# eridgd/WCT-TF

Hardware: AMD Instinct MI355X
Metric: stylized frames/sec @512x512, 5-level relu5->1 pipeline, alpha=0.8 (higher is better)
Workload: dtype f16

## Files before the change

include/wct_hip.h:

```cpp
#ifndef WCT_HIP_H
#define WCT_HIP_H

#include <stddef.h>
#include <stdint.h>

#ifdef __cplusplus
extern "C" {
#endif

typedef struct wct_ctx wct_ctx;

enum wct_status { WCT_STATUS_OK = 0, WCT_STATUS_HIP = -1, WCT_STATUS_ARG = -2,
                  WCT_STATUS_STATE = -3, WCT_STATUS_NOMEM = -4,
                  WCT_STATUS_NOCONV = -5 };

enum wct_mode { WCT_NP = 0, WCT_TF = 1 };

enum wct_flags {
  WCT_FLAG_ADAIN = 1,
  WCT_FLAG_MODE_NP = 2,
  WCT_FLAG_SWAP5 = 4,
  WCT_FLAG_STYLE_SHARED = 8,
  WCT_FLAG_IMAGES_F32 = 16,
  WCT_FLAG_CONTENT_COLORS = 32,
  WCT_FLAG_GUIDED = 64
};

int  wct_create(int device, wct_ctx** out);
void wct_destroy(wct_ctx* ctx);
const char* wct_last_error(void);
int  wct_sync(wct_ctx* ctx);
int  wct_device_count(int* n);
int  wct_get_stream(wct_ctx* ctx, void** stream_out);

int wct_set_encoder(wct_ctx* ctx, const float* pre_w, const float* pre_b,
                    const float* const* w, const float* const* b, int n_layers);
int wct_set_decoder(wct_ctx* ctx, int level, const float* const* w, const float* const* b,
                    int n_layers);

int wct_transform(wct_ctx* ctx, const float* content, int Nc, const float* style, int Ns,
                  int C, float alpha, int mode, float eps, float* out,
                  int* sweeps_out );
int wct_adain(wct_ctx* ctx, const float* content, int Nc, const float* style, int Ns,
              int C, float alpha, float epsilon, float* out);
int wct_transform_mix(wct_ctx* ctx, const float* content, int Nc, const float* const* styles, const int* Ns, int K,
                      const float* weights, int C, float alpha, int mode, float eps, float* out, int* sweeps_out);
int wct_adain_mix(wct_ctx* ctx, const float* content, int Nc, const float* const* styles, const int* Ns, int K,
                  const float* weights, int C, float alpha, float epsilon, float* out);
int wct_transform_masked(wct_ctx* ctx, const float* content, int Nc, const uint8_t* labels, const float* const* styles,
                         const int* Ns, int K, int C, float alpha, int mode, float eps, float* out, int* sweeps_out);
int wct_adain_masked(wct_ctx* ctx, const float* content, int Nc, const uint8_t* labels, const float* const* styles,
                     const int* Ns, int K, int C, float alpha, float epsilon, float* out);
int wct_mask_compact(wct_ctx* ctx, const uint8_t* mask, int Hm, int Wm, int h, int w, int stride, int K, int* perm_out,
                     int* seg_off_out);
int wct_mask_compact_batch(wct_ctx* ctx, const uint8_t* masks, int B, int Hm, int Wm, int h, int w, int stride, int K,
                           int* perm_out, int* seg_off_out);
int wct_style_swap(wct_ctx* ctx, const float* content, int hc, int wc, const float* style, int hs, int ws,
                   int C, float alpha, int patch_size, int stride, float eps, float* out);
int wct_set_style_swap(wct_ctx* ctx, float ss_alpha, int patch_size, int stride);
int wct_eigh(wct_ctx* ctx, const float* A, int C, int nmat, float* evals, float* evecs,
             int* sweeps_out );
int wct_conv3x3(wct_ctx* ctx, const float* x, int H, int W, int Cin, const float* w_hwio,
                const float* bias, int Cout, int relu, int upsample, float* y);
int wct_conv3x3_f16(wct_ctx* ctx, const float* x, int B, int H, int W, int Cin, const float* w_hwio,
                    const float* bias, int Cout, int relu, int upsample, int pool, int algo, float* y);
int wct_maxpool(wct_ctx* ctx, const float* x, int H, int W, int C, float* y);
int wct_encode(wct_ctx* ctx, const float* img01, int H, int W, int level, float* feat);
int wct_decode(wct_ctx* ctx, const float* feat, int h, int w, int level, float* img);
int wct_coral_stats(wct_ctx* ctx, const uint8_t* img, int H, int W, double sums[9]);
int wct_coral_apply(wct_ctx* ctx, const uint8_t* src, int H, int W, const double M[9],
                    const double src_mean[3], const double src_std[3],
                    const double tgt_mean[3], const double tgt_std[3],
                    uint8_t* out_u8, double* out_f64);
int wct_content_colors(wct_ctx* ctx, const uint8_t* stylized, int Ho, int Wo, const uint8_t* content, int Hc, int Wc,
                       uint8_t* out);
int wct_content_colors_batch_dev(wct_ctx* ctx, const uint8_t* stylized_dev, int Ho, int Wo, const uint8_t* content_dev, int Hc,
                                 int Wc, int B, uint8_t* out_dev);
int wct_guided_filter(wct_ctx* ctx, const uint8_t* stylized, int Ho, int Wo, const uint8_t* content, int Hc, int Wc, int radius,
                      int eps_q, uint8_t* out);
int wct_guided_filter_batch_dev(wct_ctx* ctx, const uint8_t* stylized_dev, int Ho, int Wo, const uint8_t* content_dev, int Hc, int Wc,
                                int B, int radius, int eps_q, uint8_t* out_dev);
int wct_set_guided(wct_ctx* ctx, int radius, int eps_q);
int wct_resize(wct_ctx* ctx, const uint8_t* img, int H, int W, int h, int w, uint8_t* out);
int wct_resize_batch_dev(wct_ctx* ctx, const uint8_t* in_dev, int H, int W, int B, int h, int w, uint8_t* out_dev);

int wct_output_size(int Hc, int Wc, const int* levels, int n_levels, int* Ho, int* Wo);
int wct_stylize(wct_ctx* ctx, const uint8_t* content, int Hc, int Wc,
                const uint8_t* style, int Hs, int Ws,
                const int* levels, int n_levels, float alpha, unsigned flags,
                uint8_t* out);
int wct_stylize_mix(wct_ctx* ctx, const uint8_t* content, int Hc, int Wc, const uint8_t* const* styles, const int* Hs,
                    const int* Ws, int K, const float* weights, const int* levels, int n_levels, float alpha, unsigned flags,
                    uint8_t* out);
int wct_stylize_masked(wct_ctx* ctx, const uint8_t* content, int Hc, int Wc, const uint8_t* mask, const uint8_t* const* styles,
                       const int* Hs, const int* Ws, int K, const int* levels, int n_levels, float alpha, unsigned flags,
                       uint8_t* out);
int wct_stylize_batch_dev(wct_ctx* ctx, const uint8_t* content_dev, int Hc, int Wc,
                          const uint8_t* style_dev, int Hs, int Ws, int B,
                          const int* levels, int n_levels, float alpha, unsigned flags,
                          uint8_t* out_dev);

typedef struct wct_style wct_style;
int  wct_style_prepare(wct_ctx* ctx, const uint8_t* style, int Hs, int Ws, const int* levels, int n_levels, unsigned flags,
                       wct_style** out);
void wct_style_free(wct_ctx* ctx, wct_style* style);
int  wct_stylize_prepared(wct_ctx* ctx, const uint8_t* content, int Hc, int Wc, const wct_style* style, const int* levels,
                          int n_levels, float alpha, unsigned flags, uint8_t* out);
int  wct_stylize_prepared_batch_dev(wct_ctx* ctx, const uint8_t* content_dev, int Hc, int Wc, int B, const wct_style* style,
                                    const int* levels, int n_levels, float alpha, unsigned flags, uint8_t* out_dev);
int  wct_stylize_prepared_mix(wct_ctx* ctx, const uint8_t* content, int Hc, int Wc, const wct_style* const* styles, int K,
                              const float* weights, const int* levels, int n_levels, float alpha, unsigned flags,
                              uint8_t* out);
int  wct_stylize_prepared_masked(wct_ctx* ctx, const uint8_t* content, int Hc, int Wc, const uint8_t* mask,
                                 const wct_style* const* styles, int K, const int* levels, int n_levels, float alpha,
                                 unsigned flags, uint8_t* out);
int  wct_stylize_prepared_masked_batch_dev(wct_ctx* ctx, const uint8_t* content_dev, int Hc, int Wc, int B,
                                           const uint8_t* masks_host, const wct_style* const* styles, int K, const int* levels,
                                           int n_levels, float alpha, unsigned flags, uint8_t* out_dev);

typedef struct wct_warm wct_warm;
int  wct_warm_create(wct_ctx* ctx, const int* levels, int n_levels, wct_warm** out);
void wct_warm_free(wct_ctx* ctx, wct_warm* warm);
int  wct_warm_reset(wct_ctx* ctx, wct_warm* warm);
int  wct_warm_basis(wct_ctx* ctx, const wct_warm* warm, int level, int* valid, float* V_host );
int  wct_stylize_prepared_warm(wct_ctx* ctx, const uint8_t* content, int Hc, int Wc, const wct_style* style, const int* levels,
                               int n_levels, float alpha, unsigned flags, wct_warm* warm, uint8_t* out);
int  wct_stylize_prepared_batch_dev_warm(wct_ctx* ctx, const uint8_t* content_dev, int Hc, int Wc, int B, const wct_style* style,
                                         const int* levels, int n_levels, float alpha, unsigned flags, wct_warm* warm,
                                         uint8_t* out_dev);
int  wct_transform_warm(wct_ctx* ctx, const float* content, int Nc, const float* style, int Ns, int C, float alpha,
                        unsigned flags, wct_warm* warm, int level, float* out, int* sweeps_out);

int  wct_transform_strength(wct_ctx* ctx, const float* content, int Nc, int h, int w, const uint8_t* smap, int Hm, int Wm,
                            int stride, const float* style, int Ns, int C, float alpha, int mode, float eps, float* out,
                            int* sweeps_out );
int  wct_adain_strength(wct_ctx* ctx, const float* content, int Nc, int h, int w, const uint8_t* smap, int Hm, int Wm, int stride,
                        const float* style, int Ns, int C, float alpha, float epsilon, float* out);
int  wct_stylize_prepared_strength(wct_ctx* ctx, const uint8_t* content, int Hc, int Wc, const uint8_t* smap, const wct_style* style,
                                   const int* levels, int n_levels, float alpha, unsigned flags, uint8_t* out);
int  wct_stylize_prepared_strength_batch_dev(wct_ctx* ctx, const uint8_t* content_dev, int Hc, int Wc, int B,
                                             const uint8_t* smaps_dev , const wct_style* style, const int* levels,
                                             int n_levels, float alpha, unsigned flags, uint8_t* out_dev);
int  wct_stylize_prepared_strength_batch_dev_warm(wct_ctx* ctx, const uint8_t* content_dev, int Hc, int Wc, int B,
                                                  const uint8_t* smaps_dev, const wct_style* style, const int* levels, int n_levels,
                                                  float alpha, unsigned flags, wct_warm* warm, uint8_t* out_dev);

int wct_texture_noise_batch_dev(wct_ctx* ctx, int H, int W, int B, unsigned seed, unsigned first_sample, int smooth,
                                uint8_t* out_dev);
int wct_texture_noise(wct_ctx* ctx, int H, int W, unsigned seed, unsigned sample, int smooth, uint8_t* out_host);
int wct_texture_size(int H, int W, const int* levels, int n_levels, int passes, int* Ho, int* Wo);
int wct_texture_prepared_batch_dev(wct_ctx* ctx, int H, int W, int B, unsigned seed, unsigned first_sample, int smooth,
                                   const wct_style* style, const int* levels, int n_levels, int passes, float alpha,
                                   unsigned flags, uint8_t* out_dev);
int wct_texture_prepared(wct_ctx* ctx, int H, int W, unsigned seed, unsigned sample, int smooth,
                         const wct_style* style, const int* levels, int n_levels, int passes, float alpha,
                         unsigned flags, uint8_t* out_host);

int wct_band_rows(int Hc, int Wc, const int* levels, int n_levels, int* band_rows);
int wct_band_plan(int H, int W, int level, int band_rows, int max_bands, int* n_bands, int* rows );
int wct_encode_banded(wct_ctx* ctx, const float* img01, int H, int W, int level, int band_rows, float* feat);
int wct_decode_banded(wct_ctx* ctx, const float* feat, int h, int w, int level, int band_rows, float* img);
int wct_transform_chunked(wct_ctx* ctx, const float* content, int Nc, const float* style, int Ns, int C, float alpha, int mode,
                          float eps, int chunk_rows, float* out, int* sweeps_out);
int wct_stylize_prepared_banded_dev(wct_ctx* ctx, const uint8_t* content_dev, int Hc, int Wc, const wct_style* style,
                                    const int* levels, int n_levels, float alpha, unsigned flags, int band_rows, int stat_rows,
                                    uint8_t* out_dev);
int wct_stylize_prepared_banded(wct_ctx* ctx, const uint8_t* content, int Hc, int Wc, const wct_style* style, const int* levels,
                                int n_levels, float alpha, unsigned flags, int band_rows, int stat_rows, uint8_t* out);

int wct_wrap_halo(int level, int* enc, int* dec_before, int* dec_after);
int wct_wrap_check(int H, int W, const int* levels, int n_levels);
int wct_wrap_pad_batch_dev(wct_ctx* ctx, const float* in_dev, int B, int H, int W, int C, int top, int bottom, int left, int right,
                           float* out_dev);
int wct_wrap_pad(wct_ctx* ctx, const float* x, int H, int W, int C, int top, int bottom, int left, int right, float* y);
int wct_encode_wrap(wct_ctx* ctx, const float* img01, int H, int W, int level, float* feat);
int wct_decode_wrap(wct_ctx* ctx, const float* feat, int h, int w, int level, float* img);
int wct_stylize_prepared_wrap_batch_dev(wct_ctx* ctx, const uint8_t* content_dev, int Hc, int Wc, int B, const wct_style* style,
                                        const int* levels, int n_levels, float alpha, unsigned flags, uint8_t* out_dev);
int wct_stylize_prepared_wrap(wct_ctx* ctx, const uint8_t* content, int Hc, int Wc, const wct_style* style, const int* levels,
                              int n_levels, float alpha, unsigned flags, uint8_t* out);
int wct_texture_prepared_wrap_batch_dev(wct_ctx* ctx, int H, int W, int B, unsigned seed, unsigned first_sample, int smooth,
                                        const wct_style* style, const int* levels, int n_levels, int passes, float alpha,
                                        unsigned flags, uint8_t* out_dev);
int wct_texture_prepared_wrap(wct_ctx* ctx, int H, int W, unsigned seed, unsigned sample, int smooth,
                              const wct_style* style, const int* levels, int n_levels, int passes, float alpha,
                              unsigned flags, uint8_t* out_host);

int wct_train_step(wct_ctx* ctx, int level, const float* images, int B, int H, int W,
                   float feature_weight, float pixel_weight, float tv_weight,
                   float lr, float beta1, float beta2, float eps, int step, float* losses_out);
int wct_get_decoder_layer(wct_ctx* ctx, int level, int layer, float* w_hwio, float* bias,
                          float* grad_w, float* grad_b);

int wct_train_grad_buffer(wct_ctx* ctx, int level, float** grad_dev, size_t* count);
int wct_train_apply(wct_ctx* ctx, int level, float lr, float beta1, float beta2, float eps, int step);

int wct_dev_alloc(wct_ctx* ctx, size_t bytes, void** out);
int wct_dev_free(wct_ctx* ctx, void* p);
int wct_h2d(wct_ctx* ctx, void* dst_dev, const void* src_host, size_t bytes);
int wct_d2h(wct_ctx* ctx, void* dst_host, const void* src_dev, size_t bytes);

#define WCT_PROF_CLASSES 11
int wct_prof_enable(wct_ctx* ctx, int on);
int wct_prof_reset(wct_ctx* ctx);
int wct_prof_read(wct_ctx* ctx, double ms[WCT_PROF_CLASSES], long long launches[WCT_PROF_CLASSES],
                  double flops[WCT_PROF_CLASSES], double bytes[WCT_PROF_CLASSES]);
int wct_eig_stats(wct_ctx* ctx, long long out[18]);

#ifdef __cplusplus
}
#endif
#endif
```

wct_tf_amd/_lib.py:

```python
import ctypes as C
import os

import numpy as np

_HERE = os.path.dirname(os.path.abspath(__file__))
LIB_PATH = os.path.join(_HERE, 'libwct_hip.so')

_P = C.c_void_p
_F = C.POINTER(C.c_float)
_I = C.POINTER(C.c_int)
_U8 = C.POINTER(C.c_uint8)
_D = C.POINTER(C.c_double)
_PP = C.POINTER(C.c_void_p)
SIGNATURES = [
    ('wct_create', C.c_int, [C.c_int, _PP]),
    ('wct_destroy', None, [_P]),
    ('wct_last_error', C.c_char_p, []),
    ('wct_sync', C.c_int, [_P]),
    ('wct_device_count', C.c_int, [_I]),
    ('wct_get_stream', C.c_int, [_P, _PP]),
    ('wct_set_encoder', C.c_int, [_P, _F, _F, C.POINTER(_F), C.POINTER(_F), C.c_int]),
    ('wct_set_decoder', C.c_int, [_P, C.c_int, C.POINTER(_F), C.POINTER(_F), C.c_int]),
    ('wct_transform', C.c_int, [_P, _F, C.c_int, _F, C.c_int, C.c_int, C.c_float, C.c_int, C.c_float, _F, _I]),
    ('wct_adain', C.c_int, [_P, _F, C.c_int, _F, C.c_int, C.c_int, C.c_float, C.c_float, _F]),
    ('wct_transform_mix', C.c_int, [_P, _F, C.c_int, C.POINTER(_F), _I, C.c_int, _F, C.c_int, C.c_float, C.c_int, C.c_float,
                                    _F, _I]),
    ('wct_adain_mix', C.c_int, [_P, _F, C.c_int, C.POINTER(_F), _I, C.c_int, _F, C.c_int, C.c_float, C.c_float, _F]),
    ('wct_transform_masked', C.c_int, [_P, _F, C.c_int, _U8, C.POINTER(_F), _I, C.c_int, C.c_int, C.c_float, C.c_int,
                                       C.c_float, _F, _I]),
    ('wct_adain_masked', C.c_int, [_P, _F, C.c_int, _U8, C.POINTER(_F), _I, C.c_int, C.c_int, C.c_float, C.c_float, _F]),
    ('wct_mask_compact', C.c_int, [_P, _U8, C.c_int, C.c_int, C.c_int, C.c_int, C.c_int, C.c_int, _I, _I]),
    ('wct_mask_compact_batch', C.c_int, [_P, _U8, C.c_int, C.c_int, C.c_int, C.c_int, C.c_int, C.c_int, C.c_int, _I, _I]),
    ('wct_style_swap', C.c_int, [_P, _F, C.c_int, C.c_int, _F, C.c_int, C.c_int, C.c_int, C.c_float, C.c_int, C.c_int, C.c_float, _F]),
    ('wct_set_style_swap', C.c_int, [_P, C.c_float, C.c_int, C.c_int]),
    ('wct_eigh', C.c_int, [_P, _F, C.c_int, C.c_int, _F, _F, _I]),
    ('wct_conv3x3', C.c_int, [_P, _F, C.c_int, C.c_int, C.c_int, _F, _F, C.c_int, C.c_int, C.c_int, _F]),
    ('wct_conv3x3_f16', C.c_int, [_P, _F, C.c_int, C.c_int, C.c_int, C.c_int, _F, _F, C.c_int, C.c_int, C.c_int, C.c_int, C.c_int, _F]),
    ('wct_maxpool', C.c_int, [_P, _F, C.c_int, C.c_int, C.c_int, _F]),
    ('wct_encode', C.c_int, [_P, _F, C.c_int, C.c_int, C.c_int, _F]),
    ('wct_decode', C.c_int, [_P, _F, C.c_int, C.c_int, C.c_int, _F]),
    ('wct_coral_stats', C.c_int, [_P, _U8, C.c_int, C.c_int, _D]),
    ('wct_coral_apply', C.c_int, [_P, _U8, C.c_int, C.c_int, _D, _D, _D, _D, _D, _U8, _D]),
    ('wct_content_colors', C.c_int, [_P, _U8, C.c_int, C.c_int, _U8, C.c_int, C.c_int, _U8]),
    ('wct_content_colors_batch_dev', C.c_int, [_P, _P, C.c_int, C.c_int, _P, C.c_int, C.c_int, C.c_int, _P]),
    ('wct_guided_filter', C.c_int, [_P, _U8, C.c_int, C.c_int, _U8, C.c_int, C.c_int, C.c_int, C.c_int, _U8]),
    ('wct_guided_filter_batch_dev', C.c_int, [_P, _P, C.c_int, C.c_int, _P, C.c_int, C.c_int, C.c_int, C.c_int, C.c_int, _P]),
    ('wct_set_guided', C.c_int, [_P, C.c_int, C.c_int]),
    ('wct_resize', C.c_int, [_P, _U8, C.c_int, C.c_int, C.c_int, C.c_int, _U8]),
    ('wct_resize_batch_dev', C.c_int, [_P, _P, C.c_int, C.c_int, C.c_int, C.c_int, C.c_int, _P]),
    ('wct_output_size', C.c_int, [C.c_int, C.c_int, _I, C.c_int, _I, _I]),
    ('wct_stylize', C.c_int, [_P, _U8, C.c_int, C.c_int, _U8, C.c_int, C.c_int, _I, C.c_int,
                              C.c_float, C.c_uint, _U8]),
    ('wct_stylize_mix', C.c_int, [_P, _U8, C.c_int, C.c_int, C.POINTER(_U8), _I, _I, C.c_int, _F, _I, C.c_int,
                                  C.c_float, C.c_uint, _U8]),
    ('wct_stylize_masked', C.c_int, [_P, _U8, C.c_int, C.c_int, _U8, C.POINTER(_U8), _I, _I, C.c_int, _I, C.c_int,
                                     C.c_float, C.c_uint, _U8]),
    ('wct_stylize_batch_dev', C.c_int, [_P, _P, C.c_int, C.c_int, _P, C.c_int, C.c_int, C.c_int, _I,
                                        C.c_int, C.c_float, C.c_uint, _P]),
    ('wct_style_prepare', C.c_int, [_P, _U8, C.c_int, C.c_int, _I, C.c_int, C.c_uint, _PP]),
    ('wct_style_free', None, [_P, _P]),
    ('wct_stylize_prepared', C.c_int, [_P, _U8, C.c_int, C.c_int, _P, _I, C.c_int, C.c_float, C.c_uint, _U8]),
    ('wct_stylize_prepared_batch_dev', C.c_int, [_P, _P, C.c_int, C.c_int, C.c_int, _P, _I, C.c_int, C.c_float, C.c_uint, _P]),
    ('wct_stylize_prepared_mix', C.c_int, [_P, _U8, C.c_int, C.c_int, _PP, C.c_int, _F, _I, C.c_int, C.c_float, C.c_uint, _U8]),
    ('wct_stylize_prepared_masked', C.c_int, [_P, _U8, C.c_int, C.c_int, _U8, _PP, C.c_int, _I, C.c_int, C.c_float, C.c_uint, _U8]),
    ('wct_stylize_prepared_masked_batch_dev', C.c_int, [_P, _P, C.c_int, C.c_int, C.c_int, _U8, _PP, C.c_int, _I, C.c_int, C.c_float,
                                                        C.c_uint, _P]),
    ('wct_warm_create', C.c_int, [_P, _I, C.c_int, _PP]),
    ('wct_warm_free', None, [_P, _P]),
    ('wct_warm_reset', C.c_int, [_P, _P]),
    ('wct_warm_basis', C.c_int, [_P, _P, C.c_int, _I, _F]),
    ('wct_stylize_prepared_warm', C.c_int, [_P, _U8, C.c_int, C.c_int, _P, _I, C.c_int, C.c_float, C.c_uint, _P, _U8]),
    ('wct_stylize_prepared_batch_dev_warm', C.c_int, [_P, _P, C.c_int, C.c_int, C.c_int, _P, _I, C.c_int, C.c_float, C.c_uint, _P, _P]),
    ('wct_transform_warm', C.c_int, [_P, _F, C.c_int, _F, C.c_int, C.c_int, C.c_float, C.c_uint, _P, C.c_int, _F, _I]),
    ('wct_transform_strength', C.c_int, [_P, _F, C.c_int, C.c_int, C.c_int, _U8, C.c_int, C.c_int, C.c_int, _F, C.c_int, C.c_int, C.c_float,
                                         C.c_int, C.c_float, _F, _I]),
    ('wct_adain_strength', C.c_int, [_P, _F, C.c_int, C.c_int, C.c_int, _U8, C.c_int, C.c_int, C.c_int, _F, C.c_int, C.c_int, C.c_float,
                                     C.c_float, _F]),
    ('wct_stylize_prepared_strength', C.c_int, [_P, _U8, C.c_int, C.c_int, _U8, _P, _I, C.c_int, C.c_float, C.c_uint, _U8]),
    ('wct_stylize_prepared_strength_batch_dev', C.c_int, [_P, _P, C.c_int, C.c_int, C.c_int, _P, _P, _I, C.c_int, C.c_float, C.c_uint, _P]),
    ('wct_stylize_prepared_strength_batch_dev_warm', C.c_int, [_P, _P, C.c_int, C.c_int, C.c_int, _P, _P, _I, C.c_int, C.c_float, C.c_uint,
                                                               _P, _P]),
    ('wct_texture_noise_batch_dev', C.c_int, [_P, C.c_int, C.c_int, C.c_int, C.c_uint, C.c_uint, C.c_int, _P]),
    ('wct_texture_noise', C.c_int, [_P, C.c_int, C.c_int, C.c_uint, C.c_uint, C.c_int, _U8]),
    ('wct_texture_size', C.c_int, [C.c_int, C.c_int, _I, C.c_int, C.c_int, _I, _I]),
    ('wct_texture_prepared_batch_dev', C.c_int, [_P, C.c_int, C.c_int, C.c_int, C.c_uint, C.c_uint, C.c_int, _P, _I, C.c_int, C.c_int,
                                                 C.c_float, C.c_uint, _P]),
    ('wct_texture_prepared', C.c_int, [_P, C.c_int, C.c_int, C.c_uint, C.c_uint, C.c_int, _P, _I, C.c_int, C.c_int, C.c_float,
                                       C.c_uint, _U8]),
    ('wct_band_rows', C.c_int, [C.c_int, C.c_int, _I, C.c_int, _I]),
    ('wct_band_plan', C.c_int, [C.c_int, C.c_int, C.c_int, C.c_int, C.c_int, _I, _I]),
    ('wct_encode_banded', C.c_int, [_P, _F, C.c_int, C.c_int, C.c_int, C.c_int, _F]),
    ('wct_decode_banded', C.c_int, [_P, _F, C.c_int, C.c_int, C.c_int, C.c_int, _F]),
    ('wct_transform_chunked', C.c_int, [_P, _F, C.c_int, _F, C.c_int, C.c_int, C.c_float, C.c_int, C.c_float, C.c_int, _F, _I]),
    ('wct_stylize_prepared_banded_dev', C.c_int, [_P, _P, C.c_int, C.c_int, _P, _I, C.c_int, C.c_float, C.c_uint, C.c_int, C.c_int, _P]),
    ('wct_stylize_prepared_banded', C.c_int, [_P, _U8, C.c_int, C.c_int, _P, _I, C.c_int, C.c_float, C.c_uint, C.c_int, C.c_int, _U8]),
    ('wct_wrap_halo', C.c_int, [C.c_int, _I, _I, _I]),
    ('wct_wrap_check', C.c_int, [C.c_int, C.c_int, _I, C.c_int]),
    ('wct_wrap_pad_batch_dev', C.c_int, [_P, _P, C.c_int, C.c_int, C.c_int, C.c_int, C.c_int, C.c_int, C.c_int, C.c_int, _P]),
    ('wct_wrap_pad', C.c_int, [_P, _F, C.c_int, C.c_int, C.c_int, C.c_int, C.c_int, C.c_int, C.c_int, _F]),
    ('wct_encode_wrap', C.c_int, [_P, _F, C.c_int, C.c_int, C.c_int, _F]),
    ('wct_decode_wrap', C.c_int, [_P, _F, C.c_int, C.c_int, C.c_int, _F]),
    ('wct_stylize_prepared_wrap_batch_dev', C.c_int, [_P, _P, C.c_int, C.c_int, C.c_int, _P, _I, C.c_int, C.c_float, C.c_uint, _P]),
    ('wct_stylize_prepared_wrap', C.c_int, [_P, _U8, C.c_int, C.c_int, _P, _I, C.c_int, C.c_float, C.c_uint, _U8]),
    ('wct_texture_prepared_wrap_batch_dev', C.c_int, [_P, C.c_int, C.c_int, C.c_int, C.c_uint, C.c_uint, C.c_int, _P, _I, C.c_int,
                                                      C.c_int, C.c_float, C.c_uint, _P]),
    ('wct_texture_prepared_wrap', C.c_int, [_P, C.c_int, C.c_int, C.c_uint, C.c_uint, C.c_int, _P, _I, C.c_int, C.c_int, C.c_float,
                                            C.c_uint, _U8]),
    ('wct_train_step', C.c_int, [_P, C.c_int, _F, C.c_int, C.c_int, C.c_int, C.c_float, C.c_float, C.c_float,
                                 C.c_float, C.c_float, C.c_float, C.c_float, C.c_int, _F]),
    ('wct_get_decoder_layer', C.c_int, [_P, C.c_int, C.c_int, _F, _F, _F, _F]),
    ('wct_train_grad_buffer', C.c_int, [_P, C.c_int, C.POINTER(_P), C.POINTER(C.c_size_t)]),
    ('wct_train_apply', C.c_int, [_P, C.c_int, C.c_float, C.c_float, C.c_float, C.c_float, C.c_int]),
    ('wct_dev_alloc', C.c_int, [_P, C.c_size_t, _PP]),
    ('wct_dev_free', C.c_int, [_P, _P]),
    ('wct_h2d', C.c_int, [_P, _P, _P, C.c_size_t]),
    ('wct_d2h', C.c_int, [_P, _P, _P, C.c_size_t]),
    ('wct_prof_enable', C.c_int, [_P, C.c_int]),
    ('wct_prof_reset', C.c_int, [_P]),
    ('wct_prof_read', C.c_int, [_P, _D, C.POINTER(C.c_longlong), _D, _D]),
    ('wct_eig_stats', C.c_int, [_P, C.POINTER(C.c_longlong)]),
]

WCT_NP, WCT_TF = 0, 1
FLAG_ADAIN, FLAG_MODE_NP, FLAG_SWAP5, FLAG_STYLE_SHARED, FLAG_IMAGES_F32, FLAG_CONTENT_COLORS = 1, 2, 4, 8, 16, 32
FLAG_GUIDED = 64
GUIDED_MAX_RADIUS, GUIDED_MAX_EPS = 64, 65025


def guided_eps_q(eps):
    return max(1, int(round(float(eps) * 65025)))


PROF_CLASSES = ['conv3x3', 'conv_first', 'conv_last', 'pool', 'wct_cov', 'jacobi', 'wct_apply', 'other', 'conv12', 'conv_wino', 'conv_tail']

_lib = None


class WCTHipError(RuntimeError):
    pass


class WCTNotConverged(WCTHipError):
    """WCT_STATUS_NOCONV: an eigendecomposition behind the call ran out of sweeps or met NaN/Inf (the reference's
    np.linalg.svd raises LinAlgError at the same spot, ops.py:110,123).  Outputs were written but are unreliable."""


STATUS_NOCONV = -5
MIX_MAX = 8
BATCH_MAX = 32
PASSES_MAX = 16


def load():
    global _lib
    if _lib is None:
        if not os.path.exists(LIB_PATH):
            raise WCTHipError('%s not built: run `python -m wct_tf_amd.build` (hipcc, gfx950). '
                              'There is no CPU fallback for the stylize path.' % LIB_PATH)
        lib = C.CDLL(LIB_PATH)
        for name, res, args in SIGNATURES:
            fn = getattr(lib, name)
            fn.restype = res
            fn.argtypes = args
        _lib = lib
    return _lib


def check(rc):
    if rc != 0:
        cls = WCTNotConverged if rc == STATUS_NOCONV else WCTHipError
        raise cls('libwct_hip error %d: %s' % (rc, load().wct_last_error().decode()))


def fptr(a):
    return a.ctypes.data_as(_F)


def f32(a):
    return np.ascontiguousarray(a, dtype=np.float32)


def u8(a):
    return np.ascontiguousarray(a, dtype=np.uint8)


def ptr_array(arrays):
    arr = (_F * len(arrays))(*[fptr(a) for a in arrays])
    return arr


# ... 64 lines not shown
```

wct_tf_amd/context.py:

```python
import ctypes as C

import numpy as np

from . import _lib
from ._lib import check, f32, fptr, u8
from .weights import ENCODER_CONVS, RELU_LEVEL, decoder_plan

_LEVEL_C = {1: 64, 2: 128, 3: 256, 4: 512, 5: 512}


def _levels(relu_targets):
    out = []
    for r in relu_targets:
        if isinstance(r, str):
            if r not in RELU_LEVEL:
                raise ValueError('unknown relu target %r' % (r,))
            out.append(RELU_LEVEL[r])
        else:
            out.append(int(r))
    return out


def _flags(adain=False, wct_mode='tf', swap5=False, images_f32=False, shared_style=False, content_colors=False, guided=False):
    return (_lib.FLAG_ADAIN if adain else 0) | (_lib.FLAG_MODE_NP if wct_mode == 'np' else 0) | \
# ... 329 lines not shown
                                              fptr(out), sweeps))
            return (out, list(sweeps)) if return_sweeps else out
        check(self.lib.wct_transform(self.h, fptr(c), c.shape[0], fptr(s), s.shape[0], c.shape[1],
                                     float(alpha), int(mode), float(eps), fptr(out), sweeps))
        return (out, list(sweeps)) if return_sweeps else out

    def adain(self, content, style, alpha, epsilon=1e-5):
        c = f32(content)
        s = f32(style)
        out = np.empty_like(c)
        check(self.lib.wct_adain(self.h, fptr(c), c.shape[0], fptr(s), s.shape[0], c.shape[1],
                                 float(alpha), float(epsilon), fptr(out)))
        return out

    @staticmethod
    def _strength_level(content, smap, h, w, stride):
        c = f32(content)
        m = np.asarray(smap)
        if m.ndim != 2:
            raise ValueError('expected an [H][W] strength map, got shape %s' % (m.shape,))
        m = _lib.strength_map(m, m.shape)
        if c.ndim != 2 or int(h) < 1 or int(w) < 1 or int(stride) < 1 or c.shape[0] != int(h) * int(w):
            raise ValueError('content of shape %s is not the [h*w][C] rows of a %dx%d feature map' % (c.shape, h, w))
        return c, m

    def transform_strength(self, content, style, smap, h, w, stride, alpha, mode, eps=-1.0, return_sweeps=False):
        c, m = self._strength_level(content, smap, h, w, stride)
        s = f32(style)
        if s.ndim != 2 or c.shape[1] != s.shape[1]:
            raise ValueError('expected [N][C] feature matrices with equal C')
        out = np.empty_like(c)
        sweeps = (C.c_int * 2)()
        self.last_sweeps = sweeps
        check(self.lib.wct_transform_strength(self.h, fptr(c), c.shape[0], int(h), int(w), m.ctypes.data_as(_lib._U8), m.shape[0],
                                              m.shape[1], int(stride), fptr(s), s.shape[0], c.shape[1], float(alpha), int(mode),
                                              float(eps), fptr(out), sweeps))
        return (out, list(sweeps)) if return_sweeps else out

    def adain_strength(self, content, style, smap, h, w, stride, alpha, epsilon=1e-5):
        c, m = self._strength_level(content, smap, h, w, stride)
        s = f32(style)
        out = np.empty_like(c)
        check(self.lib.wct_adain_strength(self.h, fptr(c), c.shape[0], int(h), int(w), m.ctypes.data_as(_lib._U8), m.shape[0],
                                          m.shape[1], int(stride), fptr(s), s.shape[0], c.shape[1], float(alpha), float(epsilon),
                                          fptr(out)))
        return out

    def transform_mix(self, content, styles, weights, alpha, mode, eps=-1.0, return_sweeps=False):
        c, ss, w, ns = _feature_args(content, styles, lambda c, k: _lib.mix_weights(weights, k))
        out = np.empty_like(c)
        sweeps = (C.c_int * (1 + len(ss)))()
        self.last_sweeps = sweeps
        check(self.lib.wct_transform_mix(self.h, fptr(c), c.shape[0], _lib.ptr_array(ss), ns, len(ss), fptr(w), c.shape[1],
                                         float(alpha), int(mode), float(eps), fptr(out), sweeps))
        return (out, list(sweeps)) if return_sweeps else out

    def adain_mix(self, content, styles, weights, alpha, epsilon=1e-5):
        c, ss, w, ns = _feature_args(content, styles, lambda c, k: _lib.mix_weights(weights, k))
        out = np.empty_like(c)
        check(self.lib.wct_adain_mix(self.h, fptr(c), c.shape[0], _lib.ptr_array(ss), ns, len(ss), fptr(w), c.shape[1],
                                     float(alpha), float(epsilon), fptr(out)))
        return out

    def transform_masked(self, content, styles, labels, alpha, mode, eps=-1.0, return_sweeps=False):
        c, ss, lab, ns = _feature_args(content, styles, lambda c, k: _lib.mask_labels(labels, k, (c.shape[0],)))
        out = np.empty_like(c)
        sweeps = (C.c_int * (2 * len(ss)))()
        self.last_sweeps = sweeps
        check(self.lib.wct_transform_masked(self.h, fptr(c), c.shape[0], lab.ctypes.data_as(_lib._U8), _lib.ptr_array(ss), ns,
                                            len(ss), c.shape[1], float(alpha), int(mode), float(eps), fptr(out), sweeps))
        return (out, list(sweeps)) if return_sweeps else out

    def adain_masked(self, content, styles, labels, alpha, epsilon=1e-5):
        c, ss, lab, ns = _feature_args(content, styles, lambda c, k: _lib.mask_labels(labels, k, (c.shape[0],)))
        out = np.empty_like(c)
        check(self.lib.wct_adain_masked(self.h, fptr(c), c.shape[0], lab.ctypes.data_as(_lib._U8), _lib.ptr_array(ss), ns,
                                        len(ss), c.shape[1], float(alpha), float(epsilon), fptr(out)))
        return out

    def mask_compact(self, mask, h, w, stride, k):
        m = _lib.mask_labels(mask, k)
        if m.ndim != 2:
            raise ValueError('expected an [H][W] label map')
        perm = np.empty(h * w, np.int32)
        seg = np.empty(k + 1, np.int32)
        check(self.lib.wct_mask_compact(self.h, m.ctypes.data_as(_lib._U8), m.shape[0], m.shape[1], int(h), int(w), int(stride),
                                        int(k), perm.ctypes.data_as(_lib._I), seg.ctypes.data_as(_lib._I)))
        return perm, seg

    def mask_compact_batch(self, masks, h, w, stride, k):
        m = _lib.mask_labels(masks, k)
        if m.ndim != 3:
            raise ValueError('expected [B][H][W] label maps')
        perm = np.empty((m.shape[0], h * w), np.int32)
        seg = np.empty((m.shape[0], k + 1), np.int32)
        check(self.lib.wct_mask_compact_batch(self.h, m.ctypes.data_as(_lib._U8), m.shape[0], m.shape[1], m.shape[2], int(h), int(w),
                                              int(stride), int(k), perm.ctypes.data_as(_lib._I), seg.ctypes.data_as(_lib._I)))
        return perm, seg

    def style_swap(self, content, style, alpha, patch_size=3, stride=1, eps=-1.0):
        c = f32(content)
        s = f32(style)
        out = np.empty_like(c)
        check(self.lib.wct_style_swap(self.h, fptr(c), c.shape[0], c.shape[1], fptr(s), s.shape[0], s.shape[1],
                                      c.shape[2], float(alpha), int(patch_size), int(stride), float(eps), fptr(out)))
        return out

    def set_style_swap(self, ss_alpha=0.6, patch_size=3, stride=1):
        check(self.lib.wct_set_style_swap(self.h, float(ss_alpha), int(patch_size), int(stride)))

    def eigh(self, mats, return_sweeps=False, symmetrize=True):
        a = f32(mats)
        if a.ndim == 2:
            a = a[None]
        if symmetrize:
            a = 0.5 * (a + a.transpose(0, 2, 1))
        a = np.ascontiguousarray(a, np.float32)
        n, c, _ = a.shape
        evals = np.empty((n, c), np.float32)
        evecs = np.empty((n, c, c), np.float32)
        sweeps = (C.c_int * n)()
        self.last_sweeps = sweeps
        check(self.lib.wct_eigh(self.h, fptr(a), c, n, fptr(evals), fptr(evecs), sweeps))
        return (evals, evecs, list(sweeps)) if return_sweeps else (evals, evecs)

    def conv3x3(self, x, w_hwio, bias, relu=True, upsample=False):
        x = f32(x)
        w = f32(w_hwio)
        b = f32(bias)
        h, wd, cin = x.shape
        cout = w.shape[3]
        s = 2 if upsample else 1
        y = np.empty((h * s, wd * s, cout), np.float32)
        check(self.lib.wct_conv3x3(self.h, fptr(x), h, wd, cin, fptr(w), fptr(b), cout, int(relu), int(upsample), fptr(y)))
        return y

    def conv3x3_f16(self, x, w_hwio, bias, relu=True, upsample=False, pool=False, algo=0):
        x = f32(x)
        single = x.ndim == 3
        if single:
            x = x[None]
        w = f32(w_hwio)
        b = f32(bias)
        n, h, wd, cin = x.shape
        cout = w.shape[3]
        s = 2 if upsample else 1
        ho, wo = h * s, wd * s
        if pool:
            ho, wo = (ho + 1) // 2, (wo + 1) // 2
        y = np.empty((n, ho, wo, cout), np.float32)
        check(self.lib.wct_conv3x3_f16(self.h, fptr(x), n, h, wd, cin, fptr(w), fptr(b), cout, int(relu), int(upsample), int(pool),
                                       int(algo), fptr(y)))
        return y[0] if single else y

    def maxpool(self, x):
        x = f32(x)
        h, w, c = x.shape
        y = np.empty(((h + 1) // 2, (w + 1) // 2, c), np.float32)
        check(self.lib.wct_maxpool(self.h, fptr(x), h, w, c, fptr(y)))
        return y

    def encode(self, img01, relu_target):
        level = _levels([relu_target])[0]
        x = f32(img01)
        h, w, _ = x.shape
        hh, ww = h, w
        for _ in range(level - 1):
            hh, ww = (hh + 1) // 2, (ww + 1) // 2
        feat = np.empty((hh, ww, _LEVEL_C[level]), np.float32)
        check(self.lib.wct_encode(self.h, fptr(x), h, w, level, fptr(feat)))
        return feat

    def decode(self, feat, relu_target):
        level = _levels([relu_target])[0]
        f = f32(feat)
        h, w, _ = f.shape
        s = 1 << (level - 1)
        img = np.empty((h * s, w * s, 3), np.float32)
        check(self.lib.wct_decode(self.h, fptr(f), h, w, level, fptr(img)))
        return img

    def encode_banded(self, img01, relu_target, band_rows=0):
        level = _levels([relu_target])[0]
        x = f32(img01)
        h, w, _ = x.shape
        hh, ww = h, w
        for _ in range(level - 1):
            hh, ww = (hh + 1) // 2, (ww + 1) // 2
        feat = np.empty((hh, ww, _LEVEL_C[level]), np.float32)
        check(self.lib.wct_encode_banded(self.h, fptr(x), h, w, level, int(band_rows), fptr(feat)))
        return feat

    def decode_banded(self, feat, relu_target, band_rows=0):
        level = _levels([relu_target])[0]
        f = f32(feat)
        h, w, _ = f.shape
        s = 1 << (level - 1)
        img = np.empty((h * s, w * s, 3), np.float32)
        check(self.lib.wct_decode_banded(self.h, fptr(f), h, w, level, int(band_rows), fptr(img)))
        return img

    def wrap_halo(self, relu_target):
        return wrap_halo(relu_target)

    def wrap_pad_batch_dev(self, in_dev, batch, h, w, c, pads, out_dev):
        t, b, l, r = (int(v) for v in pads)
        check(self.lib.wct_wrap_pad_batch_dev(self.h, in_dev, int(batch), int(h), int(w), int(c), t, b, l, r, out_dev))

    def wrap_pad(self, x, pads):
        a = f32(x)
        if a.ndim != 3 or a.size == 0:
            raise ValueError('wrap_pad takes an HxWxC map, got shape %s' % (a.shape,))
        t, b, l, r = (int(v) for v in pads)
        if min(t, b, l, r) < 0:
            raise ValueError('pads must be >= 0, got %r' % (pads,))
        h, w, c = a.shape
        y = np.empty((t + h + b, l + w + r, c), np.float32)
        check(self.lib.wct_wrap_pad(self.h, fptr(a), h, w, c, t, b, l, r, fptr(y)))
        return y

    def encode_wrap(self, img01, relu_target):
        level = _levels([relu_target])[0]
        x = f32(img01)
        h, w, _ = x.shape
        check_wrap(h, w, [level])
        s = 1 << (level - 1)
        feat = np.empty((h // s, w // s, _LEVEL_C[level]), np.float32)
        check(self.lib.wct_encode_wrap(self.h, fptr(x), h, w, level, fptr(feat)))
        return feat

    def decode_wrap(self, feat, relu_target):
        level = _levels([relu_target])[0]
        f = f32(feat)
        h, w, _ = f.shape
        s = 1 << (level - 1)
        img = np.empty((h * s, w * s, 3), np.float32)
        check(self.lib.wct_decode_wrap(self.h, fptr(f), h, w, level, fptr(img)))
        return img

    def transform_chunked(self, content, style, alpha, mode, chunk_rows, eps=-1.0, return_sweeps=False):
        c = f32(content)
        s = f32(style)
        if c.ndim != 2 or s.ndim != 2 or c.shape[1] != s.shape[1]:
            raise ValueError('expected [N][C] feature matrices with equal C')
        out = np.empty_like(c)
        sweeps = (C.c_int * 2)()
        self.last_sweeps = sweeps
        check(self.lib.wct_transform_chunked(self.h, fptr(c), c.shape[0], fptr(s), s.shape[0], c.shape[1], float(alpha), int(mode),
                                             float(eps), int(chunk_rows), fptr(out), sweeps))
        return (out, list(sweeps)) if return_sweeps else out

    def coral_stats(self, img_u8):
        a = u8(img_u8)
        sums = (C.c_double * 9)()
        check(self.lib.wct_coral_stats(self.h, a.ctypes.data_as(_lib._U8), a.shape[0], a.shape[1], sums))
        return np.array(list(sums), np.float64)

    def coral_apply(self, src_u8, m, src_mean, src_std, tgt_mean, tgt_std, want_f64=True, want_u8=True):
        a = u8(src_u8)
        h, w, _ = a.shape
        dd = lambda v: np.ascontiguousarray(v, np.float64).ctypes.data_as(_lib._D)
        arrs = [np.ascontiguousarray(v, np.float64).reshape(-1) for v in (m, src_mean, src_std, tgt_mean, tgt_std)]
        out8 = np.empty((h, w, 3), np.uint8) if want_u8 else None
        out64 = np.empty((h, w, 3), np.float64) if want_f64 else None
        check(self.lib.wct_coral_apply(
            self.h, a.ctypes.data_as(_lib._U8), h, w, *[x.ctypes.data_as(_lib._D) for x in arrs],
            out8.ctypes.data_as(_lib._U8) if want_u8 else None,
            out64.ctypes.data_as(_lib._D) if want_f64 else None))
        return out8, out64

    def content_colors(self, stylized_u8, content_u8):
        s, c = _color_images(stylized_u8, content_u8, 3)
        out = np.empty_like(s)
        check(self.lib.wct_content_colors(self.h, s.ctypes.data_as(_lib._U8), s.shape[0], s.shape[1], c.ctypes.data_as(_lib._U8),
                                          c.shape[0], c.shape[1], out.ctypes.data_as(_lib._U8)))
        return out

    def content_colors_batch_dev(self, stylized_dev, ho, wo, content_dev, hc, wc, batch, out_dev):
        check(self.lib.wct_content_colors_batch_dev(self.h, stylized_dev, int(ho), int(wo), content_dev, int(hc), int(wc), int(batch),
                                                    out_dev))

    def content_colors_batch(self, stylized_u8, contents_u8):
        s, c = _color_images(stylized_u8, contents_u8, 4)
        if s.shape[0] != c.shape[0] or not 1 <= s.shape[0] <= _lib.BATCH_MAX:
            raise ValueError('a batch takes 1 .. %d frames and as many contents, got %d and %d' % (_lib.BATCH_MAX, s.shape[0], c.shape[0]))
        return self._host_batch([s, c], np.empty_like(s), in_place=True, enqueue=lambda ds, dc: self.content_colors_batch_dev(
            ds, s.shape[1], s.shape[2], dc, c.shape[1], c.shape[2], s.shape[0], ds))

    def set_guided(self, radius, eps_q):
        r, e = check_guided((radius, eps_q))
        check(self.lib.wct_set_guided(self.h, r, e))

    def _set_guided(self, guided):
        if guided is None:
            return False
        self.set_guided(*check_guided(guided))
        return True

    def guided_filter(self, stylized_u8, content_u8, radius, eps_q):
        s, c = _guided_images(stylized_u8, content_u8, 3)
        r, e = check_guided((radius, eps_q))
        out = np.empty_like(s)
        check(self.lib.wct_guided_filter(self.h, s.ctypes.data_as(_lib._U8), s.shape[0], s.shape[1], c.ctypes.data_as(_lib._U8),
                                         c.shape[0], c.shape[1], r, e, out.ctypes.data_as(_lib._U8)))
        return out

# ... 514 lines not shown
```

wct_tf_amd/csrc/api_ops.hip:

```cpp
#include "api.h"

static int stage_strength(wct_ctx* c, const uint8_t* smap, int Hm, int Wm, int Nc, int h, int w, int stride, WctStrength* sm) {
  if (!smap) { wct_set_error("strength map: no map"); return WCT_ERR_ARG; }
  if (Hm < 1 || Wm < 1 || h < 1 || w < 1 || stride < 1 || (long long)h * w != Nc) {
    wct_set_error("strength map: a %dx%d map at stride %d for %d rows as %dx%d feature pixels", Hm, Wm, stride, Nc, h, w);
    return WCT_ERR_ARG;
  }
  TRY(ensure(c, c->mask_in, (size_t)Hm * Wm));
  HIP_TRY(hipMemcpyAsync(c->mask_in.p, smap, (size_t)Hm * Wm, hipMemcpyHostToDevice, c->stream));
  *sm = WctStrength{(const uint8_t*)c->mask_in.p, Hm, Wm, w, stride};
  return WCT_OK;
}

static int transform_pair(wct_ctx* c, const float* content, int Nc, const float* style, int Ns, int C, float alpha, unsigned flags,
                          float eps, wct_warm* warm, int level, float* out, int* sweeps_out, const WctStrength* sm = nullptr) {
  HIP_TRY(hipSetDevice(c->device));
  TRY(eig_stale(c));
  void *dc, *ds;
  TRY(stage_in(c, 0, content, (size_t)Nc * C * 4, &dc));
  TRY(stage_in(c, 1, style, (size_t)Ns * C * 4, &ds));
  TRY(ensure(c, c->stage[2], (size_t)Nc * C * 4));
  TRY(ensure(c, c->stage[3], 256));
  WctWarmRef wr = {};
  if (warm) {
// ... 224 lines not shown
  ARG_CHECK(c && masks && perm_out && seg_off_out && B >= 1 && B <= 32 && Hm >= 1 && Wm >= 1 && h >= 1 && w >= 1 && stride >= 1);
  TRY(mask_check(masks, (size_t)B * Hm * Wm, K));
  HIP_TRY(hipSetDevice(c->device));
  const int N = h * w;
  TRY(ensure(c, c->mask_in, (size_t)B * Hm * Wm));
  HIP_TRY(hipMemcpyAsync(c->mask_in.p, masks, (size_t)B * Hm * Wm, hipMemcpyHostToDevice, c->stream));
  const size_t perm_bytes = ((size_t)B * N * sizeof(int) + 255) & ~(size_t)255;
  const size_t seg_bytes = ((size_t)B * (WCT_MIX_MAX + 1) * sizeof(int) + 255) & ~(size_t)255;
  TRY(ensure(c, c->stage[2], perm_bytes + seg_bytes + mask_compact_workspace_bytes(N, B)));
  int* perm = (int*)c->stage[2].p;
  int* seg_off = (int*)((char*)c->stage[2].p + perm_bytes);
  TRY(launch_mask_compact_batch(MaskGeom{(const uint8_t*)c->mask_in.p, Hm, Wm, w, stride}, N, K, B, perm, seg_off, (char*)seg_off + seg_bytes,
                                c->stream));
  std::vector<int> seg((size_t)B * (WCT_MIX_MAX + 1));
  TRY(fetch(c, seg.data(), seg_off, seg.size() * sizeof(int)));
  for (int f = 0; f < B; ++f)
    for (int k = 0; k <= K; ++k) seg_off_out[f * (K + 1) + k] = seg[(size_t)f * (WCT_MIX_MAX + 1) + k];
  return fetch(c, perm_out, perm, (size_t)B * N * sizeof(int));
}

extern "C" int wct_set_style_swap(wct_ctx* c, float ss_alpha, int patch_size, int stride) {
  ARG_CHECK(c && patch_size >= 1 && stride >= 1);
  c->ss_alpha = ss_alpha; c->ss_patch = patch_size; c->ss_stride = stride;
  return WCT_OK;
}

extern "C" int wct_style_swap(wct_ctx* c, const float* content, int hc, int wc, const float* style, int hs, int ws,
                              int C, float alpha, int patch_size, int stride, float eps, float* out) {
  ARG_CHECK(c && content && style && out && hc > 0 && wc > 0 && hs > 0 && ws > 0);
  HIP_TRY(hipSetDevice(c->device));
  TRY(eig_stale(c));
  void *dc, *ds;
  TRY(stage_in(c, 0, content, (size_t)hc * wc * C * 4, &dc));
  TRY(stage_in(c, 1, style, (size_t)hs * ws * C * 4, &ds));
  TRY(ensure(c, c->stage[2], (size_t)hc * wc * C * 4));
  ARG_CHECK(patch_size >= 1 && stride >= 1 && hc >= patch_size && wc >= patch_size && hs >= patch_size && ws >= patch_size);
  TRY(ensure(c, c->wct_ws, style_swap_workspace_bytes(C, hc, wc, hs, ws, patch_size, stride)));
  TRY(launch_style_swap((float*)dc, hc, wc, (float*)ds, hs, ws, C, alpha, patch_size, stride, eps, nullptr,
                        (float*)c->stage[2].p, c->wct_ws.p, c->wct_ws.cap, c->stream, c->eig_fail_dev));
  TRY(fetch(c, out, c->stage[2].p, (size_t)hc * wc * C * 4));
  return eig_status(c);
}

__global__ void extract_diag_kernel(const float* A, float* d, int C) {
  const int m = blockIdx.y, k = blockIdx.x * blockDim.x + threadIdx.x;
  if (k < C) d[m * C + k] = A[(size_t)m * C * C + (size_t)k * C + k];
}

__global__ __launch_bounds__(256) void mirror_upper_kernel(float* A, int C) {
  __shared__ float t[32][33];
  const int bi = blockIdx.x, bj = blockIdx.y;
  if (bj < bi) return;
  float* Am = A + (size_t)blockIdx.z * C * C;
  const int tx = threadIdx.x & 31, ty = threadIdx.x >> 5;
  for (int r = ty; r < 32; r += 8) {
    const int i = bi * 32 + r, j = bj * 32 + tx;
    t[r][tx] = (i < C && j < C) ? Am[(size_t)i * C + j] : 0.f;
  }
  __syncthreads();
  for (int r = ty; r < 32; r += 8) {
    const int i = bj * 32 + r, j = bi * 32 + tx;
    if (i < C && j < C && i > j) Am[(size_t)i * C + j] = t[tx][r];
  }
}

extern "C" int wct_eigh(wct_ctx* c, const float* A, int C, int nmat, float* evals, float* evecs, int* sweeps_out) {
  ARG_CHECK(c && A && evals && evecs && nmat >= 1 && nmat <= 64 && C % 32 == 0 && C >= 32 && C <= 1024);
  HIP_TRY(hipSetDevice(c->device));
  TRY(eig_stale(c));
  const size_t mb = (size_t)nmat * C * C * 4;
  void* dA;
  TRY(stage_in(c, 0, A, mb, &dA));
  hipLaunchKernelGGL(mirror_upper_kernel, dim3(cdiv(C, 32), cdiv(C, 32), nmat), dim3(256), 0, c->stream, (float*)dA, C);
  TRY(ensure(c, c->stage[1], mb));
  TRY(ensure(c, c->stage[2], (size_t)nmat * C * 4 + 1024));
  TRY(ensure(c, c->wct_ws, jacobi_workspace_bytes(C, nmat)));
  int* sw = (int*)((char*)c->stage[2].p + (size_t)nmat * C * 4);
  {
    ProfScope ps(c, 5, 0, 0);
    TRY(launch_jacobi_eigh((float*)dA, (float*)c->stage[1].p, C, nmat, c->wct_ws.p, c->wct_ws.cap, sw, c->eig_fail_dev, c->stream));
  }
  hipLaunchKernelGGL(extract_diag_kernel, dim3(cdiv(C, 256), nmat), dim3(256), 0, c->stream, (float*)dA, (float*)c->stage[2].p, C);
  TRY(fetch(c, evals, c->stage[2].p, (size_t)nmat * C * 4));
  TRY(fetch(c, evecs, c->stage[1].p, mb));
  if (sweeps_out) TRY(fetch(c, sweeps_out, sw, nmat * sizeof(int)));
  return eig_status(c);
}

extern "C" int wct_conv3x3(wct_ctx* c, const float* x, int H, int W, int Cin, const float* w_hwio, const float* bias,
                           int Cout, int relu, int upsample, float* y) {
  ARG_CHECK(c && x && w_hwio && bias && y);
  HIP_TRY(hipSetDevice(c->device));
  const int Ho = upsample ? 2 * H : H, Wo = upsample ? 2 * W : W;
  ConvLayer l;
  TRY(pack_conv(c, w_hwio, bias, Cin, Cout, &l));
  void* dx;
  int rc = stage_in(c, 0, x, (size_t)H * W * Cin * 4, &dx);
  if (!rc) rc = ensure(c, c->stage[1], (size_t)H * W * Cin * 2);
  if (!rc) rc = ensure(c, c->stage[2], (size_t)Ho * Wo * Cout * 4);
  if (!rc) rc = launch_f32_to_f16((float*)dx, (half_t*)c->stage[1].p, (size_t)H * W * Cin, c->stream);
  if (!rc) rc = run_conv(c, l, (half_t*)c->stage[1].p, nullptr, (float*)c->stage[2].p, 1, Ho, Wo, upsample, relu);
  if (!rc) rc = fetch(c, y, c->stage[2].p, (size_t)Ho * Wo * Cout * 4);
  hipStreamSynchronize(c->stream);
  free_layer(l);
  return rc;
}

extern "C" int wct_conv3x3_f16(wct_ctx* c, const float* x, int B, int H, int W, int Cin, const float* w_hwio, const float* bias,
                               int Cout, int relu, int upsample, int pool, int algo, float* y) {
  ARG_CHECK(c && x && w_hwio && bias && y && B >= 1 && algo >= 0 && algo <= 2);
  HIP_TRY(hipSetDevice(c->device));
  const int Hc = upsample ? 2 * H : H, Wc = upsample ? 2 * W : W;
  const int Ho = pool ? (Hc + 1) / 2 : Hc, Wo = pool ? (Wc + 1) / 2 : Wc;
  ConvLayer l;
  TRY(pack_conv(c, w_hwio, bias, Cin, Cout, &l));
  int rc = WCT_OK;
  if (algo == 2 && !l.ww) {
    float* w32 = nullptr;
    rc = upload(c, w_hwio, (size_t)9 * Cin * Cout * sizeof(float), (void**)&w32);
    if (!rc && hipMalloc((void**)&l.ww, (size_t)Cout * 12 * Cin * sizeof(half_t)) != hipSuccess) { wct_set_error("hipMalloc failed"); rc = WCT_ERR_NOMEM; }
    if (!rc) rc = launch_pack_conv_wino_frag(w32, l.ww, Cin, Cout, c->stream);
    hipStreamSynchronize(c->stream);
    if (w32) hipFree(w32);
  }
  const bool keep = c->no_wino;
  c->no_wino = algo == 1;
  void* dx;
  const size_t nin = (size_t)B * H * W * Cin, nout = (size_t)B * Ho * Wo * Cout;
  if (!rc) rc = stage_in(c, 0, x, nin * 4, &dx);
  if (!rc) rc = ensure(c, c->stage[1], nin * 2);
  if (!rc) rc = ensure(c, c->stage[2], nout * 2);
  if (!rc) rc = ensure(c, c->stage[3], nout * 4);
  if (!rc) rc = launch_f32_to_f16((float*)dx, (half_t*)c->stage[1].p, nin, c->stream);
  if (!rc) {
    ConvArgs a;
    a.x = (half_t*)c->stage[1].p; a.w = l.w; a.bias = l.b; a.y16 = (half_t*)c->stage[2].p; a.y32 = nullptr; a.usum = nullptr; a.umax = nullptr;
    a.B = B; a.H = Hc; a.W = Wc; a.Cin = Cin; a.Cout = Cout; a.upsample = upsample; a.relu = relu; a.pool = pool;
    a.w_wino = c->no_wino ? nullptr : l.ww;
    if (algo == 2 && !conv3x3_wino_takes(a)) { wct_set_error("wct_conv3x3_f16: algo 2 does not take this layer"); rc = WCT_ERR_ARG; }
    if (!rc) {
      const double px = (double)B * Hc * Wc;
      ProfScope ps(c, 0, 2.0 * px * 9 * Cin * Cout, (double)nin * 2 + (double)nout * 2 + 9.0 * Cin * Cout * 2);
      rc = launch_conv3x3(a, c->stream);
    }
  }
  c->no_wino = keep;
  if (!rc) rc = launch_f16_to_f32((half_t*)c->stage[2].p, (float*)c->stage[3].p, nout, c->stream);
  if (!rc) rc = fetch(c, y, c->stage[3].p, nout * 4);
  hipStreamSynchronize(c->stream);
  free_layer(l);
  return rc;
}

extern "C" int wct_maxpool(wct_ctx* c, const float* x, int H, int W, int C, float* y) {
  ARG_CHECK(c && x && y && C % 8 == 0);
  HIP_TRY(hipSetDevice(c->device));
  const int Ho = (H + 1) / 2, Wo = (W + 1) / 2;
  void* dx;
  TRY(stage_in(c, 0, x, (size_t)H * W * C * 4, &dx));
  TRY(ensure(c, c->stage[1], (size_t)H * W * C * 2));
  TRY(ensure(c, c->stage[2], (size_t)Ho * Wo * C * 2));
  TRY(ensure(c, c->stage[3], (size_t)Ho * Wo * C * 4));
  TRY(launch_f32_to_f16((float*)dx, (half_t*)c->stage[1].p, (size_t)H * W * C, c->stream));
  TRY(launch_maxpool2x2((half_t*)c->stage[1].p, (half_t*)c->stage[2].p, 1, H, W, C, c->stream));
  TRY(launch_f16_to_f32((half_t*)c->stage[2].p, (float*)c->stage[3].p, (size_t)Ho * Wo * C, c->stream));
  return fetch(c, y, c->stage[3].p, (size_t)Ho * Wo * C * 4);
}

extern "C" int wct_encode(wct_ctx* c, const float* img01, int H, int W, int level, float* feat) {
  ARG_CHECK(c && img01 && feat && level >= 1 && level <= 5);
  HIP_TRY(hipSetDevice(c->device));
  TRY(check_min_size("image", H, W, level));
  int h, w;
  level_dims(H, W, level, &h, &w);
  void* dimg;
  TRY(stage_in(c, 0, img01, (size_t)H * W * 3 * 4, &dimg));
  const size_t fb = (size_t)h * w * LEVEL_C[level] * 4;
  TRY(ensure(c, c->feat_c, fb));
  float* taps[6] = {};
  taps[level] = (float*)c->feat_c.p;
  TRY(run_encoder(c, (float*)dimg, 1, H, W, 0, level, taps));
  return fetch(c, feat, c->feat_c.p, fb);
}

extern "C" int wct_decode(wct_ctx* c, const float* feat, int h, int w, int level, float* img) {
  ARG_CHECK(c && feat && img && level >= 1 && level <= 5);
  HIP_TRY(hipSetDevice(c->device));
  const int C = LEVEL_C[level], scale = 1 << (level - 1);
  void* df;
  TRY(stage_in(c, 0, feat, (size_t)h * w * C * 4, &df));
  TRY(ensure(c, c->wct_out, (size_t)h * w * C * 2));
  TRY(launch_f32_to_f16((float*)df, (half_t*)c->wct_out.p, (size_t)h * w * C, c->stream));
  const size_t ib = (size_t)h * scale * w * scale * 3 * 4;
  TRY(ensure(c, c->img_t[0], ib));
  TRY(run_decoder(c, level, (half_t*)c->wct_out.p, 1, h, w, (float*)c->img_t[0].p));
  return fetch(c, img, c->img_t[0].p, ib);
}

static int twin_band_rows(int H, int W, int level, int* band_rows) {
  Chain chain;
  TRY(chain_geometry(H, W, &level, 1, &chain));
  if (*band_rows) return band_rows_check(chain, *band_rows);
  TRY(band_rows_for(chain, band_rows));
  if (!*band_rows) *band_rows = (H + 15) / 16 * 16;
  return WCT_OK;
}

extern "C" int wct_encode_banded(wct_ctx* c, const float* img01, int H, int W, int level, int band_rows, float* feat) {
  ARG_CHECK(c && img01 && feat && level >= 1 && level <= 5 && band_rows >= 0);
  HIP_TRY(hipSetDevice(c->device));
  TRY(twin_band_rows(H, W, level, &band_rows));
  int h, w;
  level_dims(H, W, level, &h, &w);
  void* dimg;
  TRY(stage_in(c, 0, img01, (size_t)H * W * 3 * 4, &dimg));
  const size_t fb = (size_t)h * w * LEVEL_C[level] * 4;
  TRY(ensure(c, c->band_f, fb));
  TRY(run_encoder_banded(c, (float*)dimg, H, W, 0, level, band_rows, (float*)c->band_f.p));
  return fetch(c, feat, c->band_f.p, fb);
}

extern "C" int wct_decode_banded(wct_ctx* c, const float* feat, int h, int w, int level, int band_rows, float* img) {
  ARG_CHECK(c && feat && img && level >= 1 && level <= 5 && band_rows >= 0 && h >= 2 && w >= 2 && h <= (1 << 26) && w <= (1 << 26));
  HIP_TRY(hipSetDevice(c->device));
  const int C = LEVEL_C[level], scale = 1 << (level - 1);
  TRY(twin_band_rows(h * scale, w * scale, level, &band_rows));
  void* df;
  const size_t n = (size_t)h * w * C;
  TRY(stage_in(c, 0, feat, n * 4, &df));
  TRY(ensure(c, c->band_g, n * 2));
  TRY(launch_f32_to_f16((float*)df, (half_t*)c->band_g.p, n, c->stream));
  const size_t ib = (size_t)h * scale * w * scale * 3 * 4;
  TRY(ensure(c, c->img_t[0], ib));
  TRY(run_decoder_banded(c, level, (half_t*)c->band_g.p, h, w, band_rows, (float*)c->img_t[0].p));
  return fetch(c, img, c->img_t[0].p, ib);
}

extern "C" int wct_wrap_pad_batch_dev(wct_ctx* c, const float* in, int B, int H, int W, int C, int top, int bottom, int left, int right,
                                      float* out) {
  ARG_CHECK(c != nullptr);
  if (!in || !out) { wct_set_error("wrap pad: null map pointer"); return WCT_ERR_ARG; }
  if (B < 1 || B > 32) { wct_set_error("wrap pad: B = %d maps, must be 1 .. 32", B); return WCT_ERR_ARG; }
  if (H < 1 || W < 1 || C < 1 || top < 0 || bottom < 0 || left < 0 || right < 0) {
    wct_set_error("wrap pad: a %dx%dx%d map with pads %d %d %d %d (sizes >= 1, pads >= 0)", H, W, C, top, bottom, left, right);
    return WCT_ERR_ARG;
  }
  HIP_TRY(hipSetDevice(c->device));
  ProfScope ps(c, 7, 0, 2.0 * B * ((double)top + H + bottom) * ((double)left + W + right) * C * 4);
  return launch_wrap_pad(in, out, B, H, W, C, 4, top, bottom, left, right, c->stream);
}

extern "C" int wct_wrap_pad(wct_ctx* c, const float* x, int H, int W, int C, int top, int bottom, int left, int right, float* y) {
  ARG_CHECK(c && x && y && H >= 1 && W >= 1 && C >= 1 && top >= 0 && bottom >= 0 && left >= 0 && right >= 0);
  HIP_TRY(hipSetDevice(c->device));
  const unsigned long long out_elems = ((unsigned long long)top + H + bottom) * ((unsigned long long)left + W + right) * (unsigned long long)C;
  if (out_elems >= (1ull << 29)) {
    wct_set_error("wrap pad: the padded %dx%dx%d map passes 2^31 bytes in one launch", H, W, C);
    return WCT_ERR_ARG;
  }
  void* dx;
  TRY(stage_in(c, 0, x, (size_t)H * W * C * 4, &dx));
  TRY(ensure(c, c->stage[1], (size_t)out_elems * 4));
  TRY(wct_wrap_pad_batch_dev(c, (const float*)dx, 1, H, W, C, top, bottom, left, right, (float*)c->stage[1].p));
  return fetch(c, y, c->stage[1].p, (size_t)out_elems * 4);
}

extern "C" int wct_encode_wrap(wct_ctx* c, const float* img01, int H, int W, int level, float* feat) {
  ARG_CHECK(c && img01 && feat && level >= 1 && level <= 5);
  HIP_TRY(hipSetDevice(c->device));
  Chain chain;
  TRY(wrap_chain_check(H, W, &level, 1, &chain));
  void* dimg;
  TRY(stage_in(c, 0, img01, (size_t)H * W * 3 * 4, &dimg));
  const size_t fb = (size_t)chain.lv[0].h * chain.lv[0].w * LEVEL_C[level] * 4;
  TRY(ensure(c, c->wrap_f, fb));
  TRY(run_encoder_wrap(c, (const float*)dimg, 1, H, W, 0, level, (float*)c->wrap_f.p));
  return fetch(c, feat, c->wrap_f.p, fb);
}

extern "C" int wct_decode_wrap(wct_ctx* c, const float* feat, int h, int w, int level, float* img) {
  ARG_CHECK(c && feat && img && level >= 1 && level <= 5 && h >= 1 && w >= 1 && h <= (1 << 26) && w <= (1 << 26));
  HIP_TRY(hipSetDevice(c->device));
  const int C = LEVEL_C[level], scale = 1 << (level - 1);
  Chain chain;
  TRY(wrap_chain_check(h * scale, w * scale, &level, 1, &chain));
  void* df;
  const size_t n = (size_t)h * w * C;
  TRY(stage_in(c, 0, feat, n * 4, &df));
  TRY(ensure(c, c->wct_out, n * 2));
  TRY(launch_f32_to_f16((float*)df, (half_t*)c->wct_out.p, n, c->stream));
  const size_t ib = (size_t)h * scale * w * scale * 3 * 4;
  TRY(ensure(c, c->img_t[0], ib));
  TRY(run_decoder_wrap(c, level, (const half_t*)c->wct_out.p, 1, h, w, (float*)c->img_t[0].p));
  return fetch(c, img, c->img_t[0].p, ib);
}

extern "C" int wct_coral_stats(wct_ctx* c, const uint8_t* img, int H, int W, double sums[9]) {
  ARG_CHECK(c && img && sums && H > 0 && W > 0);
  HIP_TRY(hipSetDevice(c->device));
  const size_t npix = (size_t)H * W;
  void* dimg;
  TRY(stage_in(c, 0, img, npix * 3, &dimg));
  int nblocks = (int)((npix + 255) / 256);
  if (nblocks > 1024) nblocks = 1024;
  TRY(ensure(c, c->stage[1], (size_t)(nblocks + 1) * 9 * sizeof(unsigned long long)));
  unsigned long long* partial = (unsigned long long*)c->stage[1].p;
// ... 174 lines not shown
```

wct_tf_amd/csrc/common.h:

```cpp
#pragma once
#include <hip/hip_runtime.h>
#include <stdint.h>
#include <stddef.h>
#include "skip_rule.h"

typedef _Float16 half_t;
typedef _Float16 half8 __attribute__((ext_vector_type(8)));
typedef _Float16 half4 __attribute__((ext_vector_type(4)));
typedef float f32x16 __attribute__((ext_vector_type(16)));
typedef float f32x4 __attribute__((ext_vector_type(4)));

#define WCT_OK 0
#define WCT_ERR_HIP -1
#define WCT_ERR_ARG -2
#define WCT_ERR_STATE -3
#define WCT_ERR_NOMEM -4
#define WCT_ERR_NOCONV -5

void wct_set_error(const char* fmt, ...);

#define HIP_TRY(expr)                                                          \
  do {                                                                         \
    hipError_t _e = (expr);                                                    \
    if (_e != hipSuccess) {                                                    \
      wct_set_error("%s failed: %s (%s:%d)", #expr, hipGetErrorString(_e),     \
                    __FILE__, __LINE__);                                       \
      return WCT_ERR_HIP;                                                      \
    }                                                                          \
  } while (0)

#define ARG_CHECK(cond)                                                        \
  do {                                                                         \
    if (!(cond)) {                                                             \
      wct_set_error("invalid argument: %s (%s:%d)", #cond, __FILE__, __LINE__);\
      return WCT_ERR_ARG;                                                      \
    }                                                                          \
  } while (0)

static inline int cdiv(int a, int b) { return (a + b - 1) / b; }

constexpr size_t WCT_LAUNCH_BYTES = (size_t)1 << 31;
static inline bool launch_map_fits(size_t elems, size_t bytes) { return elems * bytes < WCT_LAUNCH_BYTES; }


struct ConvArgs {
  const half_t* x;
  const half_t* w;
  const float* bias;
  half_t* y16;
  float* y32;
  int B, H, W;
  int Cin, Cout;
  int upsample;
  int relu;
  int pool;
  float* usum;
  unsigned* umax;
  const float* img1 = nullptr;
  const half_t* w1frag = nullptr;
  const float* bias1 = nullptr;
  int clamp01 = 0;
  const half_t* w_wino = nullptr;
};
constexpr int UMAX_SLOTS = 64;
__device__ __forceinline__ void umax_merge(unsigned* umax_img, int slot, float vmax, int lane) {
#pragma unroll
  for (int o = 32; o > 0; o >>= 1) vmax = fmaxf(vmax, __shfl_xor(vmax, o, 64));
  if (lane == 0) {
    unsigned* w = umax_img + (slot & (UMAX_SLOTS - 1));
    const unsigned bits = __builtin_bit_cast(unsigned, vmax);
    if (bits > __atomic_load_n(w, __ATOMIC_RELAXED)) atomicMax(w, bits);
  }
}
int launch_conv3x3(const ConvArgs& a, hipStream_t s);
bool conv3x3_wino_takes(const ConvArgs& a);
int launch_conv3x3_wino(const ConvArgs& a, hipStream_t s);

struct ConvFirstArgs {
  const float* x;
  const half_t* wfrag;
  const float* bias;
  half_t* y16;
  float* y32;
  int B, H, W;
  int clamp01;
  float* usum;
  unsigned* umax;
};

__device__ __forceinline__ void unit_row_sum4(f32x4& t) {
  float a = t[0], b = t[1], c = t[2], d = t[3];
#define WCT_DPP_STEP(ctrl)                                                             \
  "v_add_f32_dpp %0, %0, %0 " ctrl " row_mask:0xf bank_mask:0xf bound_ctrl:1\n"       \
  "v_add_f32_dpp %1, %1, %1 " ctrl " row_mask:0xf bank_mask:0xf bound_ctrl:1\n"       \
  "v_add_f32_dpp %2, %2, %2 " ctrl " row_mask:0xf bank_mask:0xf bound_ctrl:1\n"       \
  "v_add_f32_dpp %3, %3, %3 " ctrl " row_mask:0xf bank_mask:0xf bound_ctrl:1\n"
  asm volatile("s_nop 1\n"
               WCT_DPP_STEP("quad_perm:[1,0,3,2]")
               WCT_DPP_STEP("quad_perm:[2,3,0,1]")
               WCT_DPP_STEP("row_half_mirror")
               WCT_DPP_STEP("row_mirror")
               : "+v"(a), "+v"(b), "+v"(c), "+v"(d));
#undef WCT_DPP_STEP
  t[0] = a; t[1] = b; t[2] = c; t[3] = d;
}
int launch_conv_first(const ConvFirstArgs& a, hipStream_t s);

struct ConvLastArgs {
  const half_t* x;
  const half_t* wfrag;
  const float* bias;
  float* y;
  int B, H, W;
};
int launch_conv_last(const ConvLastArgs& a, hipStream_t s);

int launch_maxpool2x2(const half_t* x, half_t* y, int B, int H, int W, int C, hipStream_t s);
int launch_u8_to_f32(const uint8_t* x, float* y, size_t n, hipStream_t s);
int launch_f32_to_u8(const float* x, uint8_t* y, size_t n, hipStream_t s);
int launch_f32_to_f16(const float* x, half_t* y, size_t n, hipStream_t s);
int launch_f16_to_f32(const half_t* x, float* y, size_t n, hipStream_t s);

struct GemmArgs {
  const float* A; int lda; int a_kmajor;
  const float* B; int ldb; int b_kmajor;
  const float* a_sub_m;
  const float* b_sub_n;
  const float* a_sub_k;
  const float* a_scale_k;
  int M, N, K;
  int ksplit;
  float* out32; half_t* out16; int ldo;
  size_t out_split_stride;
  const float* bias_n;
  int nsplit;
  size_t sA, sB, s_sub_m, s_sub_n, s_sub_k, s_scale_k, s_out, s_bias;
  const float* A_odd;
  size_t sA_odd;
  WctSkip skip;
  int blend; float alpha; unsigned* mabs;
  const float* mask_diag; size_t s_mask; int* mask_out; const int* mask_in;
};

int launch_gemm(GemmArgs g, int nsplit, int nbatch, hipStream_t s);

enum { WCT_MODE_NP = 0, WCT_MODE_TF = 1 };

struct WctFeatStats { const float* u[2]; const unsigned* umax[2]; };

struct WctStyleKey { int nslab, nsplit, ksplit; };
WctStyleKey wct_style_key(int C, int Nc, int Ns);
size_t wct_style_state_floats(int C);
size_t wct_style_workspace_bytes(int C, int Ns, const WctStyleKey& key);
struct WctStyleRef { const float* state[8]; };
struct WctStyleSlots { const float* state[32]; };

struct WctWarmRef { float* basis; int valid; };

struct WctStrength { const uint8_t* smap; int Hm, Wm, w, stride; };

struct WctCall {
  float alpha; int mode;
  float eps;
  half_t* out16; float* out32;
  void* workspace; size_t workspace_bytes;
  int* sweeps_dev;
  int stages;
  int* eig_fail;
  hipStream_t stream;
};
enum { WCT_STAGE_COV = 1, WCT_STAGE_EIG = 2, WCT_STAGE_APPLY = 4, WCT_STAGE_ALL = 7, WCT_STAGE_EIG_FP32UPDATE = 8 };

int launch_style_state(const float* style, int Ns, int C, const WctStyleKey& key, int adain, const WctCall& r, float* state);

size_t wct_workspace_bytes(int C, int Nc, int Ns, int P);
int launch_wct(const float* content, int Nc, const float* style, int Ns, int C, int P, WctSkip skip, const WctCall& r,
               const WctFeatStats* stats, const WctStyleRef* prep, const WctWarmRef* warm, const WctStrength* sm = nullptr);
int launch_adain(const float* content, int Nc, const float* style, int Ns, int C, int P, WctSkip skip, const WctCall& r,
                 const WctFeatStats* stats, const WctStyleRef* prep, const WctStrength* sm = nullptr);
enum { WCT_MIX_MAX = 8 };
size_t wct_mix_workspace_bytes(int C, int Nc, const int* Ns, int K, const float* lambda);
int launch_wct_mix(const float* content, int Nc, const float* const* styles, const int* Ns, int K, const float* lambda, int C,
                   const WctCall& r, const WctFeatStats* stats, const WctStyleRef* prep);
int launch_adain_mix(const float* content, int Nc, const float* const* styles, const int* Ns, int K, const float* lambda, int C,
                     const WctCall& r, const WctFeatStats* stats, const WctStyleRef* prep);
struct MaskGeom { const uint8_t* mask; int Hm, Wm, w, stride; };
size_t mask_compact_workspace_bytes(int N, int G = 1);
int launch_mask_compact(const MaskGeom& g, int N, int K, int* perm, int* seg_off, void* workspace, hipStream_t s);
size_t wct_masked_workspace_bytes(int C, int Nc, const int* nk, const int* Ns, int K);
int launch_wct_masked(const float* content, int Nc, const MaskGeom& g, const int* nk, const float* const* styles, const int* Ns, int K,
                      int C, const WctCall& r);
int launch_adain_masked(const float* content, int Nc, const MaskGeom& g, const int* nk, const float* const* styles, const int* Ns, int K,
                        int C, const WctCall& r);
size_t wct_masked_batch_workspace_bytes(int C, int Nc, int G, const int* nk, const int* Ns, int K);
int wct_masked_batch_pairs(int G, const int* nk, int K);
int launch_mask_compact_batch(const MaskGeom& g, int N, int K, int G, int* perm, int* seg_off, void* workspace, hipStream_t s);
int launch_wct_masked_batch(const float* content, int Nc, int G, const MaskGeom& g, const int* nk, const int* Ns, int K, int C,
                            const WctCall& r, const WctStyleSlots& states);
int launch_adain_masked_batch(const float* content, int Nc, int G, const MaskGeom& g, const int* nk, const int* Ns, int K, int C,
                              const WctCall& r, const WctStyleSlots& states);
int launch_jacobi_eigh(float* A, float* V, int C, int nmat, void* workspace,
                       size_t workspace_bytes, int* sweeps_done_dev, int* eig_fail, hipStream_t s);
size_t jacobi_workspace_bytes(int C, int nmat);

size_t style_swap_workspace_bytes(int C, int hc, int wc, int hs, int ws, int patch, int stride);
int launch_style_swap(const float* content, int hc, int wc, const float* style, int hs, int ws, int C,
                      float alpha, int patch, int stride, float eps, half_t* out16, float* out32,
                      void* workspace, size_t workspace_bytes, hipStream_t s, int* eig_fail);

int launch_im2col_act(const half_t* x, float* col, int B, int H, int W, int C, int upsample, hipStream_t s);
int launch_im2col_grad(const float* g, float* col, int B, int H, int W, int C, hipStream_t s);
int launch_reflect_fold(const float* gp, float* g, int B, int H, int W, int C, hipStream_t s);
int launch_relu_mask16(float* g, const half_t* act, size_t n, hipStream_t s);
int launch_relu_mask32(float* g, const float* act, size_t n, hipStream_t s);
int launch_upsample_adjoint(const float* gb, float* gs, int B, int h, int w, int C, hipStream_t s);
int launch_maxpool_adjoint(const half_t* pre, const float* gpool, float* gpre, int B, int H, int W, int C, hipStream_t s);
int launch_mse(const float* a, const float* b, size_t n, float weight, float* grad, int accumulate, double* partial,
               float* loss_out, hipStream_t s);
int launch_tv(const float* x, int B, int H, int W, int C, float weight, float* grad, double* partial, float* loss_out, hipStream_t s);
int launch_bias_grad(const float* g, size_t rows, int C, float* partial, float* out, hipStream_t s);
int launch_reduce_slabs(const float* partial, size_t n, int nslab, float* out, hipStream_t s);
int launch_adam(float* w, float* m, float* v, const float* g, size_t n, float lr_t, float b1, float b2, float eps, hipStream_t s);
int launch_pack_conv_frag(const float* w, half_t* frag, int cin, int cout, hipStream_t s);
int launch_pack_conv_wino_frag(const float* w, half_t* frag, int cin, int cout, hipStream_t s);
int launch_pack_last_frag(const float* w, half_t* frag, hipStream_t s);
int launch_transpose_w(const float* w, float* wt, int cin, int cout, int cout_pad, hipStream_t s);
int launch_pad3to4(const float* x, float* y, size_t n, hipStream_t s);
int launch_conv_dgrad(const float* g, const float* wt, int B, int H, int W, int cin, int cout,
                      float* col, float* gp, float* gin, void* scratch, hipStream_t s);
int launch_conv_wgrad(const half_t* x16, int upsample, const float* g, int ldg, int B, int H, int W, int cin, int cout,
                      float* col, float* partial, int nsplit, float* dw, void* scratch, hipStream_t s);
int conv_wgrad_splits(int B, int H, int W);
int launch_pow2_scale(const float* x, size_t n, void* scratch, hipStream_t s);
int launch_conv_first_dgrad(const float* g, const float* wf, float* gp, int B, int H, int W, hipStream_t s);

struct CoralApplyArgs {
  double M[9], src_mean[3], src_std[3], tgt_mean[3], tgt_std[3];
};
int launch_coral_stats(const uint8_t* img, size_t npix, unsigned long long* partial, int nblocks,
                       unsigned long long* out9, hipStream_t s);
int launch_coral_apply(const uint8_t* src, size_t npix, const CoralApplyArgs& a, uint8_t* out_u8,
                       double* out_f64, hipStream_t s);

int launch_content_colors_f32(const float* frame, const void* content, int content_f32, int B, int Ho, int Wo, int Hc, int Wc,
                              uint8_t* out, hipStream_t s);
int launch_content_colors_u8(const uint8_t* stylized, const uint8_t* content, int B, int Ho, int Wo, int Hc, int Wc, uint8_t* out,
                             hipStream_t s);
int launch_content_colors_u8_any(const uint8_t* stylized, const void* content, int content_f32, int B, int Ho, int Wo, int Hc, int Wc,
                                 uint8_t* out, hipStream_t s);

int guided_check(int B, int Ho, int Wo, int Hc, int Wc, int radius, int eps_q);
size_t guided_workspace_bytes(int B, int Ho, int Wo);
int launch_guided_filter(const uint8_t* stylized, const void* content, int content_f32, int B, int Ho, int Wo, int Hc, int Wc, int radius,
                         int eps_q, void* workspace, uint8_t* out, hipStream_t s);

int launch_texture_noise(uint8_t* out, int B, int H, int W, unsigned seed, unsigned first_sample, int smooth, hipStream_t s);

int launch_wrap_pad(const void* in, void* out, int B, int H, int W, int E, int elem_bytes, int t, int b, int l, int r, hipStream_t s);
int launch_wrap_crop(const void* in, void* out, int B, int Hp, int Wp, int E, int elem_bytes, int t, int l, int h, int w, hipStream_t s);

struct ResizeGeom { int H, W, h, w, ksx, ksy, th; };
int resize_check_bytes(int B, int H, int W, int h, int w);
size_t resize_table_ints(int H, int W, int h, int w);
int resize_plan(int H, int W, int h, int w, ResizeGeom* g, int* tabs);
int launch_resize(const uint8_t* in, uint8_t* out, int B, const ResizeGeom& g, const int* tabs_dev, hipStream_t s);
```

wct_tf_amd/csrc/spectral.hip:

```cpp
#include "wct_stages.h"

__device__ __forceinline__ bool pair_resolved(float dp, float dq, float e) { return e * e <= 0.25f * dp * dq; }

constexpr float SPECTRAL_NOISE_CUT = 2.f;
__device__ __forceinline__ float spectral_cut(const float* Am, int C, int tid, float* red) {
  float mn = 0.f;
  for (int i = tid; i < C; i += 256) mn = fminf(mn, Am[(size_t)i * C + i]);
  for (int o = 32; o > 0; o >>= 1) mn = fminf(mn, __shfl_xor(mn, o, 64));
  if ((tid & 63) == 0) red[tid >> 6] = mn;
  __syncthreads();
  mn = fminf(fminf(red[0], red[1]), fminf(red[2], red[3]));
  return fmaxf(1e-5f, -SPECTRAL_NOISE_CUT * mn);
}

__device__ __forceinline__ float spectral_entry(float dp, float dq, float e, bool diag, int kind, float shift, float cut) {
  const bool kp = dp > cut, kq = dq > cut;
  if (diag) return kp ? (kind == 0 ? 1.f / sqrtf(dp + shift) : sqrtf(dp + shift)) : 0.f;
  if (!kp && !kq) return 0.f;
  if (kp && kq) {
    if (!pair_resolved(dp, dq, e)) return 0.f;
    const float sa = sqrtf(dp + shift), sb = sqrtf(dq + shift);
    return kind == 0 ? -e / (sa * sb * (sa + sb)) : e / (sa + sb);
  }
  const float dk = kp ? dp : dq, dd = kp ? dq : dp;
  const float fk = kind == 0 ? 1.f / sqrtf(dk + shift) : sqrtf(dk + shift);
  return e * fk / fmaxf(dk - dd, 2.f * fabsf(e));
}

struct SpectralTile {
  float dp[64], dq[64];
  float mt[64][65];
};
__attribute__((used)) __device__ __forceinline__ void spectral_tile_load(SpectralTile& t, const float* Am, int C, int p0, int q0, int tid) {
  if (tid < 64) t.dp[tid] = p0 + tid < C ? Am[(size_t)(p0 + tid) * C + p0 + tid] : 0.f;
  else if (tid < 128) t.dq[tid - 64] = q0 + tid - 64 < C ? Am[(size_t)(q0 + tid - 64) * C + q0 + tid - 64] : 0.f;
  const int ty = tid >> 4, tx = tid & 15;
#pragma unroll
  for (int i = 0; i < 4; ++i) {
    const int r = q0 + ty * 4 + i, c = p0 + tx * 4;
    f32x4 v = {0.f, 0.f, 0.f, 0.f};
    if (r < C && c < C) v = *reinterpret_cast<const f32x4*>(Am + (size_t)r * C + c);
#pragma unroll
    for (int j = 0; j < 4; ++j) t.mt[ty * 4 + i][tx * 4 + j] = v[j];
  }
}

struct SpecAllArgs {
  const float* A;
  float* G;
  float *N, *R, *Pm;
  const float *X1, *X2;
  int C; float shift; int correct, second; WctSkip skip;
  unsigned* mabs; const float* mean; float* bias; float alpha; int mode;
};

__global__ __launch_bounds__(256) void spectral_open_all_kernel(SpecAllArgs a) {
  __shared__ SpectralTile t;
  const int m = blockIdx.z, p0 = blockIdx.y * 64, q0 = blockIdx.x * 64, tid = threadIdx.x;
  const int C = a.C, kind = m & 1, pair = m >> 1;
  const size_t cc = (size_t)C * C;
  if (kind == 0 && blockIdx.x == 0 && blockIdx.y == 0) {
    if (tid == 0) a.mabs[pair] = 0u;
    const float* mp = a.mean + (size_t)(one_content(a.skip) ? 0 : pair) * 2 * C;
    const float* ms = a.mean + (size_t)(one_style(a.skip) ? 0 : pair) * 2 * C + C;
    for (int i = tid; i < C; i += 256) {
      float b = a.alpha * ms[i];
      if (a.mode == WCT_MODE_TF) b += (1.f - a.alpha) * mp[i];
      a.bias[pair * C + i] = b;
    }
  }
  if (skip_style_mat(m, a.skip)) return;
  __shared__ float cutred[4];
  const float* Am = a.A + m * cc;
  const float cut = spectral_cut(Am, C, tid, cutred);
  spectral_tile_load(t, Am, C, p0, q0, tid);
  __syncthreads();
  const int ty = tid >> 4, tx = tid & 15;
#pragma unroll
  for (int i = 0; i < 4; ++i) {
    const int pl = ty * 4 + i, p = p0 + pl, q = q0 + tx * 4;
    if (p >= C || q >= C) continue;
    const f32x4 av = *reinterpret_cast<const f32x4*>(Am + (size_t)p * C + q);
    const float dp = t.dp[pl];
    f32x4 g, n4 = {0.f, 0.f, 0.f, 0.f}, r4 = n4, p4 = n4;
#pragma unroll
    for (int j = 0; j < 4; ++j) {
      const float dk = t.dq[tx * 4 + j];
      const float em = 0.5f * (av[j] + t.mt[tx * 4 + j][pl]);
      g[j] = spectral_entry(dp, dk, a.correct ? em : 0.f, p == q + j, kind, a.shift, cut);
      if (a.second && p != q + j && dp > cut && dk > cut && pair_resolved(dp, dk, em)) {
        const float sp = sqrtf(dp + a.shift), sk = sqrtf(dk + a.shift);
        n4[j] = em / (sp + sk);
        r4[j] = em / sk;
        p4[j] = n4[j] / sk;
      }
    }
    const size_t o = (size_t)p * C + q;
    *reinterpret_cast<f32x4*>(a.G + m * cc + o) = g;
    if (a.second) {
      *reinterpret_cast<f32x4*>(a.N + m * cc + o) = n4;
      if (kind == 0) { *reinterpret_cast<f32x4*>(a.R + pair * cc + o) = r4; *reinterpret_cast<f32x4*>(a.Pm + pair * cc + o) = p4; }
    }
  }
}

__global__ __launch_bounds__(256) void spectral_add2_all_kernel(SpecAllArgs a) {
  __shared__ float dps[64], dqs[64];
  __shared__ float x1t[64][65], x2t[64][65];
  const int m = blockIdx.z, p0 = blockIdx.y * 64, q0 = blockIdx.x * 64, tid = threadIdx.x;
  if (skip_style_mat(m, a.skip)) return;
  const int C = a.C, kind = m & 1;
  const size_t cc = (size_t)C * C;
  const float* Am = a.A + m * cc;
  float* Gm = a.G + m * cc;
  const float* X2 = a.X2 + m * cc;
  const float* X1 = a.X1 + (size_t)(m >> 1) * cc;
  int near = 0;
  for (int i = tid; i < C; i += 256) {
    const float d = fabsf(Am[(size_t)i * C + i]);
    near |= (d > 3.3e-6f) & (d < 3e-5f);
  }
  if (__syncthreads_or(near)) return;
  __shared__ float cutred[4];
  const float cut = spectral_cut(Am, C, tid, cutred);
  if (tid < 64) dps[tid] = p0 + tid < C ? Am[(size_t)(p0 + tid) * C + p0 + tid] : 0.f;
  else if (tid < 128) dqs[tid - 64] = q0 + tid - 64 < C ? Am[(size_t)(q0 + tid - 64) * C + q0 + tid - 64] : 0.f;
  const int ty = tid >> 4, tx = tid & 15;
#pragma unroll
  for (int i = 0; i < 4; ++i) {
    const int r = q0 + ty * 4 + i, c = p0 + tx * 4;
    f32x4 v1 = {0.f, 0.f, 0.f, 0.f}, v2 = v1;
    if (r < C && c < C) {
      v2 = *reinterpret_cast<const f32x4*>(X2 + (size_t)r * C + c);
      if (kind == 0) v1 = *reinterpret_cast<const f32x4*>(X1 + (size_t)r * C + c);
    }
#pragma unroll
    for (int j = 0; j < 4; ++j) { x2t[ty * 4 + i][tx * 4 + j] = v2[j]; x1t[ty * 4 + i][tx * 4 + j] = v1[j]; }
  }
  __syncthreads();
#pragma unroll
  for (int i = 0; i < 4; ++i) {
    const int pl = ty * 4 + i, p = p0 + pl, q = q0 + tx * 4;
    if (p >= C || q >= C) continue;
    const size_t o = (size_t)p * C + q;
    const f32x4 x2 = *reinterpret_cast<const f32x4*>(X2 + o);
    f32x4 x1 = {0.f, 0.f, 0.f, 0.f};
    if (kind == 0) x1 = *reinterpret_cast<const f32x4*>(X1 + o);
    f32x4 g = *reinterpret_cast<const f32x4*>(Gm + o);
    const float dp = dps[pl];
#pragma unroll
    for (int j = 0; j < 4; ++j) {
      const float dq = dqs[tx * 4 + j];
      if (!(dp > cut && dq > cut)) continue;
      const float sp = sqrtf(dp + a.shift), sq = sqrtf(dq + a.shift);
      float l2;
      if (kind == 1) l2 = -0.5f * (x2[j] + x2t[tx * 4 + j][pl]) / (sp + sq);
      else l2 = (0.5f * (x1[j] + x1t[tx * 4 + j][pl]) + 0.25f * (sp + sq) * (x2[j] + x2t[tx * 4 + j][pl])) / (sp * sq * (sp + sq));
      g[j] += l2;
    }
    *reinterpret_cast<f32x4*>(Gm + o) = g;
  }
}

static GemmArgs level_product(int C, WctSkip skip) {
  GemmArgs g = {};
  g.lda = g.ldb = g.ldo = C; g.M = g.N = g.K = g.ksplit = C; g.sA = g.sB = g.s_out = (size_t)C * C; g.skip = skip;
  return g;
}

static int launch_refresh(const WctCarve& w, int C, int P, WctSkip skip, hipStream_t s) {
  int rc;
  GemmArgs r1 = level_product(C, skip);
  r1.A = w.A0; r1.a_kmajor = 0; r1.B = w.V; r1.b_kmajor = 1; r1.out32 = w.X;
  r1.mask_diag = w.A; r1.s_mask = (size_t)C * C; r1.mask_out = w.refresh;
  if ((rc = launch_gemm(r1, 1, 2 * P, s))) return rc;
  GemmArgs r2 = level_product(C, skip);
  r2.A = w.V; r2.a_kmajor = 1; r2.B = w.X; r2.b_kmajor = 1; r2.out32 = w.A; r2.mask_in = w.refresh;
  return launch_gemm(r2, 1, 2 * P, s);
}

int launch_spectral_tail_refreshed(const WctCarve& w, int C, int P, float alpha, int mode, float eps_in, WctSkip skip, int nwhite,
                                   hipStream_t s) {
  int rc;
  const size_t cc = (size_t)C * C;
  const float shift = mode == WCT_MODE_NP ? (eps_in >= 0.f ? eps_in : 1e-5f) : 0.f;
  const int second = EIG_CORRECT >= 2;
  const dim3 tiles(cdiv(C, 64), cdiv(C, 64), 2 * P);
  SpecAllArgs sa = {};
  sa.A = w.A; sa.G = w.G; sa.C = C; sa.shift = shift; sa.correct = EIG_CORRECT; sa.second = second; sa.skip = skip;
  sa.N = w.S2; float* X2 = sa.N + 2 * P * cc; sa.R = X2 + 2 * P * cc; sa.Pm = sa.R + P * cc; float* X1 = sa.Pm + P * cc;
  sa.X1 = X1; sa.X2 = X2;
  sa.mabs = w.mabs; sa.mean = w.mean; sa.bias = w.bias; sa.alpha = alpha; sa.mode = mode;
  hipLaunchKernelGGL(spectral_open_all_kernel, tiles, dim3(256), 0, s, sa);
  HIP_TRY(hipGetLastError());
  if (second) {
    GemmArgs a = level_product(C, skip);
    a.A = sa.Pm; a.A_odd = sa.N + cc; a.sA_odd = 2 * cc; a.a_kmajor = 0; a.B = sa.N; a.b_kmajor = 1; a.out32 = X2;
    if ((rc = launch_gemm(a, 1, 2 * P, s))) return rc;
    GemmArgs b = level_product(C, WCT_SKIP_NONE);
    b.A = sa.R; b.a_kmajor = 0; b.B = sa.N; b.b_kmajor = 1; b.sB = 2 * cc; b.out32 = X1;
    if (nwhite > 0 && (rc = launch_gemm(b, 1, nwhite, s))) return rc;
    hipLaunchKernelGGL(spectral_add2_all_kernel, tiles, dim3(256), 0, s, sa);
    HIP_TRY(hipGetLastError());
  }
  GemmArgs g = level_product(C, skip);
  g.A = w.V; g.a_kmajor = 0; g.B = w.G; g.b_kmajor = 1; g.out32 = w.X;
  if ((rc = launch_gemm(g, 1, 2 * P, s))) return rc;
  GemmArgs h = level_product(C, skip);
  h.A = w.X; h.a_kmajor = 0; h.B = w.V; h.b_kmajor = 0; h.out32 = w.Tw;
  return launch_gemm(h, 1, 2 * P, s);
}

int launch_spectral_tail(const WctCarve& w, int C, int P, float alpha, int mode, float eps_in, WctSkip skip, int nwhite,
                         hipStream_t s) {
  const int rc = launch_refresh(w, C, P, skip, s);
  return rc ? rc : launch_spectral_tail_refreshed(w, C, P, alpha, mode, eps_in, skip, nwhite, s);
}
```

wct_tf_amd/csrc/stats_gemm.hip:

```cpp
#include "wct_stages.h"


struct StatArgs {
  const float* x[2];
  int n[2];
  const float* u[2];
  const unsigned* umax[2];
  const float* mean;
  float* partial;
  float* absmax;
  int C, nslab;
  WctSkip skip;
};

__global__ __launch_bounds__(256) void colsum_kernel(StatArgs p) {
  __shared__ f32x4 red[256];
  const int mat = blockIdx.y, slab = blockIdx.x;
  if (skip_style_mat(mat, p.skip)) return;
  const int b = mat & 1, pair = mat >> 1;
  const int C = p.C, cq = C / 4;
  const int nrp = 256 / cq;
  const int tid = threadIdx.x;
  const int rp = tid / cq, c4 = tid % cq;
  const int N = p.n[b];
// ... 388 lines not shown
    }
  } else {
    if (kbeg < kend) { load(ra, voff_a, kbeg); load(rb, voff_b, kbeg); }
    for (int k0 = kbeg; k0 < kend; k0 += 32) {
      if (k0 + 32 <= kend) {
        split_store(ra, mean_a, k0, false, lds[0], lds[1]);
        split_store(rb, mean_b, k0, false, lds[2], lds[3]);
      } else {
        split_store(ra, mean_a, k0, true, lds[0], lds[1]);
        split_store(rb, mean_b, k0, true, lds[2], lds[3]);
      }
      __syncthreads();
      if (k0 + 32 < kend) { load(ra, voff_a, k0 + 32); load(rb, voff_b, k0 + 32); }
      mma_stage(lds[2], lds[3]);
      __syncthreads();
    }
  }

  float* out = p.partial + ((size_t)mat * p.nsplit + split) * C * C;
#pragma unroll
  for (int i = 0; i < TM; ++i)
#pragma unroll
    for (int j = 0; j < TM; ++j) {
      const int gn = n0 + (wn * TM + j) * 32 + (lane & 31);
#pragma unroll
      for (int r = 0; r < 16; ++r) {
        const int gm = m0 + (wm * TM + i) * 32 + (r & 3) + 8 * (r >> 2) + 4 * (lane >> 5);
        if (gm < C && gn < C) out[(size_t)gm * C + gn] = acc[i][j][r];
      }
    }
}

__global__ __launch_bounds__(256) void cov_finish_kernel(const float* partial, const float* scale, float* cov, int C, int nsplit, int BT,
                                                         float inv0, float inv1, float eps, int skip, float* cov0 = nullptr) {
  __shared__ float tt[64][65];
  const int mat = blockIdx.z;
  if (skip_style_mat(mat, skip)) return;
  const size_t cc = (size_t)C * C;
  const int r0 = blockIdx.y * 64, c0 = blockIdx.x * 64, tid = threadIdx.x, ty = tid >> 4, tx = tid & 15;
  const bool mirror = r0 / BT > c0 / BT;
  const float* pb = partial + (size_t)mat * nsplit * cc;
  const float sc = scale[mat];
  const float f = ((mat & 1) == 0 ? inv0 : inv1) / (sc * sc);
  f32x4 acc[4];
#pragma unroll
  for (int i = 0; i < 4; ++i) {
    const int r = (mirror ? c0 : r0) + ty * 4 + i, c = (mirror ? r0 : c0) + tx * 4;
    f32x4 sum = {0.f, 0.f, 0.f, 0.f};
    if (r < C && c < C)
      for (int k = 0; k < nsplit; ++k) sum += *reinterpret_cast<const f32x4*>(pb + (size_t)k * cc + (size_t)r * C + c);
    acc[i] = sum;
  }
  if (mirror) {
#pragma unroll
    for (int i = 0; i < 4; ++i)
#pragma unroll
      for (int j = 0; j < 4; ++j) tt[ty * 4 + i][tx * 4 + j] = acc[i][j];
    __syncthreads();
#pragma unroll
    for (int i = 0; i < 4; ++i)
#pragma unroll
      for (int j = 0; j < 4; ++j) acc[i][j] = tt[tx * 4 + j][ty * 4 + i];
  }
#pragma unroll
  for (int i = 0; i < 4; ++i) {
    const int r = r0 + ty * 4 + i, c = c0 + tx * 4;
    if (r >= C || c >= C) continue;
    f32x4 v = acc[i] * f;
#pragma unroll
    for (int j = 0; j < 4; ++j) if (r == c + j) v[j] += eps;
    *reinterpret_cast<f32x4*>(cov + (size_t)mat * cc + (size_t)r * C + c) = v;
    if (cov0) *reinterpret_cast<f32x4*>(cov0 + (size_t)mat * cc + (size_t)r * C + c) = v;
  }
}

static int stat_passes(StatArgs sa, int nmat, float* mean, float* var, float* scale, float d0, float d1, hipStream_t s) {
  const int C = sa.C;
  sa.mean = nullptr;
  hipLaunchKernelGGL(colsum_kernel, dim3(sa.nslab, nmat), dim3(256), 0, s, sa);
  hipLaunchKernelGGL(colsum_finish_kernel, dim3(cdiv(C, 256), nmat), dim3(256), 0, s, sa.partial, mean, C, sa.nslab, d0, d1, (int)sa.skip,
                     (const float*)sa.absmax, scale);
  if (var) {
    sa.mean = mean; sa.absmax = nullptr;
    hipLaunchKernelGGL(colsum_kernel, dim3(sa.nslab, nmat), dim3(256), 0, s, sa);
    hipLaunchKernelGGL(colsum_finish_kernel, dim3(cdiv(C, 256), nmat), dim3(256), 0, s, sa.partial, var, C, sa.nslab, d0, d1, (int)sa.skip,
                       (const float*)nullptr, (float*)nullptr);
  }
  HIP_TRY(hipGetLastError());
  return WCT_OK;
}

int launch_means(const float* content, int Nc, const float* style, int Ns, int C, int P, const WctCarve& w, bool with_var, WctSkip skip,
                 hipStream_t s, const WctFeatStats* fs) {
  StatArgs sa;
  sa.x[0] = content; sa.x[1] = style; sa.n[0] = Nc; sa.n[1] = Ns;
  for (int b = 0; b < 2; ++b) {
    sa.u[b] = fs && fs->umax[b] ? fs->u[b] : nullptr;
    sa.umax[b] = sa.u[b] ? fs->umax[b] : nullptr;
  }
  sa.partial = w.stat_partial; sa.absmax = w.absmax; sa.C = C; sa.nslab = w.nslab; sa.skip = skip;
  return stat_passes(sa, 2 * P, w.mean, with_var ? w.var : nullptr, w.scale, (float)Nc, (float)Ns, s);
}

static int cov_passes(CovArgs ca, int nmat, float* A, float* A0, float inv0, float inv1, float eps, hipStream_t s) {
  const int C = ca.C, BT = C >= 128 ? 128 : 64;
  ca.ntile = cdiv(C, BT);
  dim3 grid(ca.ntile * (ca.ntile + 1) / 2, ca.nsplit, nmat);
  if (BT == 128) hipLaunchKernelGGL((cov_f16x2_kernel<128>), grid, dim3(256), 0, s, ca);
  else hipLaunchKernelGGL((cov_f16x2_kernel<64>), grid, dim3(256), 0, s, ca);
  hipLaunchKernelGGL(cov_finish_kernel, dim3(cdiv(C, 64), cdiv(C, 64), nmat), dim3(256), 0, s, ca.partial, ca.scale, A, C, ca.nsplit, BT,
                     inv0, inv1, eps, (int)ca.skip, A0);
  HIP_TRY(hipGetLastError());
  return WCT_OK;
}

int launch_cov(const float* content, int Nc, const float* style, int Ns, int C, int P, const WctCarve& w, float eps, WctSkip skip,
               hipStream_t s) {
  CovArgs ca;
  ca.x[0] = content; ca.x[1] = style; ca.n[0] = Nc; ca.n[1] = Ns;
  ca.mean = w.mean; ca.scale = w.scale; ca.partial = w.cov_partial;
  ca.C = C; ca.ksplit = w.ksplit; ca.nsplit = w.nsplit; ca.skip = skip;
  return cov_passes(ca, 2 * P, w.A, w.A0, 1.f / (float)(Nc - 1), 1.f / (float)(Ns - 1), eps, s);
}

static int launch_slot_means(const float* x, int N, int C, int m, int nslab, const WctCarve& w, bool with_var, hipStream_t s,
                             const float* u, const unsigned* umax) {
  StatArgs sa = {};
  sa.x[0] = sa.x[1] = x; sa.n[0] = sa.n[1] = N;
  sa.u[0] = umax ? u : nullptr; sa.umax[0] = sa.u[0] ? umax : nullptr;
  sa.partial = w.stat_partial + (size_t)m * w.nslab * C; sa.absmax = w.absmax + (size_t)m * w.nslab;
  sa.C = C; sa.nslab = nslab; sa.skip = WCT_SKIP_NONE;
  return stat_passes(sa, 1, w.mean + (size_t)m * C, with_var ? w.var + (size_t)m * C : nullptr, w.scale + m, (float)N, (float)N, s);
}

static int launch_slot_cov(const float* x, int N, int C, int m, int nsplit, int ksplit, float eps, const WctCarve& w, hipStream_t s) {
  const size_t cc = (size_t)C * C;
  CovArgs ca;
  ca.x[0] = ca.x[1] = x; ca.n[0] = ca.n[1] = N;
  ca.mean = w.mean + (size_t)m * C; ca.scale = w.scale + m; ca.partial = w.cov_partial + (size_t)m * w.nsplit * cc;
  ca.C = C; ca.ksplit = ksplit; ca.nsplit = nsplit; ca.skip = WCT_SKIP_NONE;
  return cov_passes(ca, 1, w.A + m * cc, w.A0 + m * cc, 1.f / (float)(N - 1), 1.f / (float)(N - 1), eps, s);
}

int launch_plan_stats(const SlotPlan& sp, int C, bool with_var, bool with_cov, float eps, hipStream_t s) {
  int rc;
  for (int m = 0; m < 2 * sp.P; ++m) {
    const SlotPlan::Slot& t = sp.slot[m];
    if (!t.n) continue;
    if ((rc = launch_slot_means(t.x, t.n, C, m, t.lay.nslab, sp.w, with_var, s, m ? nullptr : sp.u0, m ? nullptr : sp.umax0))) return rc;
    if (with_cov && (rc = launch_slot_cov(t.x, t.n, C, m, t.lay.nsplit, t.lay.ksplit, eps, sp.w, s))) return rc;
  }
  return WCT_OK;
}
```

wct_tf_amd/csrc/style_swap.hip:

```cpp
#include "wct_stages.h"

__global__ void im2col_kernel(const float* src, float* dst, int w, int C, int p, int st, int ho, int wo) {
  const int c4n = C / 4;
  const size_t total = (size_t)ho * wo * p * p * c4n;
  for (size_t e = blockIdx.x * (size_t)blockDim.x + threadIdx.x; e < total; e += (size_t)gridDim.x * blockDim.x) {
    const int c4 = (int)(e % c4n);
    size_t t = e / c4n;
    const int j = (int)(t % p); t /= p;
    const int i = (int)(t % p); t /= p;
    const int x = (int)(t % wo), y = (int)(t / wo);
    reinterpret_cast<f32x4*>(dst)[e] =
        *reinterpret_cast<const f32x4*>(src + ((size_t)(y * st + i) * w + (x * st + j)) * C + c4 * 4);
  }
}

__global__ void patch_axis_inv_norm_kernel(const float* B, float* inv, int n, int K) {
  const int k4 = blockIdx.x * blockDim.x + threadIdx.x;
  if (k4 * 4 >= K) return;
  f32x4 s = {0.f, 0.f, 0.f, 0.f};
  for (int r = 0; r < n; ++r) {
    const f32x4 v = *reinterpret_cast<const f32x4*>(B + (size_t)r * K + k4 * 4);
    s += v * v;
  }
  f32x4 o;
#pragma unroll
  for (int j = 0; j < 4; ++j) o[j] = 1.f / sqrtf(fmaxf(s[j], 1e-12f));
  *reinterpret_cast<f32x4*>(inv + k4 * 4) = o;
}

__global__ __launch_bounds__(64) void row_argmax_kernel(const float* E, int* idx, int n) {
  const int m = blockIdx.x, lane = threadIdx.x;
  float best = -INFINITY;
  int bi = 0x7fffffff;
  for (int j = lane; j < n; j += 64) {
    const float v = E[(size_t)m * n + j];
    if (v > best) { best = v; bi = j; }
  }
  for (int o = 32; o > 0; o >>= 1) {
    const float ob = __shfl_xor(best, o, 64);
    const int oi = __shfl_xor(bi, o, 64);
    if (ob > best || (ob == best && oi < bi)) { best = ob; bi = oi; }
  }
  if (lane == 0) idx[m] = (bi >= 0 && bi < n) ? bi : 0;
}

__global__ void swap_reconstruct_kernel(const float* patches , const int* idx, float* out,
                                        int h, int w, int C, int p, int st, int ho, int wo) {
  const int c4n = C / 4;
  const size_t total = (size_t)h * w * c4n;
  for (size_t e = blockIdx.x * (size_t)blockDim.x + threadIdx.x; e < total; e += (size_t)gridDim.x * blockDim.x) {
    const int c4 = (int)(e % c4n);
    const size_t pix = e / c4n;
    const int x = (int)(pix % w), y = (int)(pix / w);
    f32x4 acc = {0.f, 0.f, 0.f, 0.f};
    float cnt = 0.f;
    for (int i = 0; i < p; ++i) {
      const int yy = y - i;
      if (yy < 0 || yy % st) continue;
      const int py = yy / st;
      if (py >= ho) continue;
      for (int j = 0; j < p; ++j) {
        const int xx = x - j;
        if (xx < 0 || xx % st) continue;
        const int px = xx / st;
        if (px >= wo) continue;
        const int n = idx[py * wo + px];
        acc += *reinterpret_cast<const f32x4*>(patches + ((size_t)n * p * p + i * p + j) * C + c4 * 4);
        cnt += 1.f;
      }
    }
    reinterpret_cast<f32x4*>(out)[e] = acc / cnt;
  }
}

__global__ void swap_blend_kernel(const float* col, const float* x, const float* ms, size_t n4, int C, float alpha,
                                  half_t* out16, float* out32) {
  const int cq = C / 4;
  for (size_t i = blockIdx.x * (size_t)blockDim.x + threadIdx.x; i < n4; i += (size_t)gridDim.x * blockDim.x) {
    const int c = (int)(i % cq) * 4;
    const f32x4 a = reinterpret_cast<const f32x4*>(col)[i], b = reinterpret_cast<const f32x4*>(x)[i];
    const f32x4 m = *reinterpret_cast<const f32x4*>(ms + c);
    const f32x4 o = alpha * (a + m) + (1.f - alpha) * b;
    if (out32) reinterpret_cast<f32x4*>(out32)[i] = o;
    if (out16) {
      half4 h;
#pragma unroll
      for (int j = 0; j < 4; ++j) h[j] = (half_t)o[j];
      reinterpret_cast<half4*>(out16)[i] = h;
    }
  }
}

struct SwapCarve {
  float *d3, *Wc, *Ws, *Ac, *Bs, *inv, *E, *ss, *col;
  int* idx;
  size_t total;
};

static SwapCarve swap_carve(void* base, int C, int hc, int wc, int hs, int ws, int p, int st) {
  SwapCarve w;
  const size_t K = (size_t)p * p * C;
  const size_t Mo = (size_t)((hc - p) / st + 1) * ((wc - p) / st + 1);
  const size_t Pn = (size_t)((hs - p) / st + 1) * ((ws - p) / st + 1);
  size_t off = 0;
  char* b = reinterpret_cast<char*>(base);
  auto take = [&](size_t bytes) { void* q = b ? b + off : nullptr; off += align_up(bytes); return q; };
  w.d3 = (float*)take(3 * (size_t)C * 4);
  w.Wc = (float*)take((size_t)hc * wc * C * 4);
  w.Ws = (float*)take((size_t)hs * ws * C * 4);
  w.Ac = (float*)take(Mo * K * 4);
  w.Bs = (float*)take(Pn * K * 4);
  w.inv = (float*)take(K * 4);
  w.E = (float*)take(Mo * Pn * 4);
  w.idx = (int*)take(Mo * 4);
  w.ss = (float*)take((size_t)hc * wc * C * 4);
  w.col = (float*)take((size_t)hc * wc * C * 4);
  w.total = off;
  return w;
}

size_t style_swap_workspace_bytes(int C, int hc, int wc, int hs, int ws, int p, int st) {
  return wct_workspace_bytes(C, hc * wc, hs * ws, 1) + swap_carve(nullptr, C, hc, wc, hs, ws, p, st).total + 1024;
}

static inline unsigned ew_grid(size_t n) { size_t g = (n + 255) / 256; return (unsigned)(g > 4096 ? 4096 : (g ? g : 1)); }

int launch_style_swap(const float* content, int hc, int wc, const float* style, int hs, int ws, int C,
                      float alpha, int patch, int stride, float eps, half_t* out16, float* out32,
                      void* workspace, size_t workspace_bytes, hipStream_t s, int* eig_fail) {
  ARG_CHECK(C % 32 == 0 && C >= 32 && C <= 1024 && patch >= 1 && stride >= 1);
  ARG_CHECK(hc >= patch && wc >= patch && hs >= patch && ws >= patch);
  const int ho = (hc - patch) / stride + 1, wo = (wc - patch) / stride + 1;
  const int rows = (hs - patch) / stride + 1, cols = (ws - patch) / stride + 1;
  if ((ho - 1) * stride + patch != hc || (wo - 1) * stride + patch != wc) {
    wct_set_error("style-swap with patch %d stride %d maps a %dx%d feature map to %dx%d: pre-size the content "
                  "(swap_filter_fit / center_crop_to, wct.py:84-90)", patch, stride, hc, wc,
                  (ho - 1) * stride + patch, (wo - 1) * stride + patch);
    return WCT_ERR_ARG;
  }
  const int Nc = hc * wc, Ns = hs * ws, Mo = ho * wo, Pn = rows * cols, K = patch * patch * C;
  const size_t wct_bytes = align_up(wct_workspace_bytes(C, Nc, Ns, 1));
  ARG_CHECK(workspace_bytes >= style_swap_workspace_bytes(C, hc, wc, hs, ws, patch, stride));
  WctCarve w = carve(workspace, C, 1, pair_layout(C, Nc, Ns));
  SwapCarve sw = swap_carve((char*)workspace + wct_bytes, C, hc, wc, hs, ws, patch, stride);
  int rc;
  WctCall r = {};
  r.alpha = alpha; r.mode = WCT_MODE_TF; r.eps = eps; r.workspace = workspace; r.workspace_bytes = wct_bytes;
  r.stages = WCT_STAGE_COV | WCT_STAGE_EIG | WCT_STAGE_EIG_FP32UPDATE; r.eig_fail = eig_fail; r.stream = s;
  if ((rc = launch_wct(content, Nc, style, Ns, C, 1, WCT_SKIP_NONE, r, nullptr, nullptr, nullptr))) return rc;
  const size_t cc = (size_t)C * C;
  if ((rc = launch_spectral_tail(w, C, 1, alpha, WCT_MODE_TF, eps, WCT_SKIP_NONE, 1, s))) return rc;
  WctCarve v = w;
  v.A += cc; v.V += cc; v.G += cc; v.X += cc; v.Tw = w.T;
  if ((rc = launch_spectral_tail_refreshed(v, C, 1, alpha, WCT_MODE_TF, eps, WCT_SKIP_STYLE, 1, s))) return rc;
  auto apply = [&](const float* X, int N, const float* mean, const float* T, float* out) {
    GemmArgs g = {};
    g.A = X; g.lda = C; g.a_kmajor = 0; g.a_sub_k = mean; g.B = T; g.ldb = C; g.b_kmajor = 0;
    g.M = N; g.N = C; g.K = C; g.ksplit = C; g.out32 = out; g.ldo = C;
    return launch_gemm(g, 1, 1, s);
  };
  if ((rc = apply(content, Nc, w.mean, w.Tw, sw.Wc))) return rc;
  if ((rc = apply(style, Ns, w.mean + C, w.T, sw.Ws))) return rc;
  hipLaunchKernelGGL(im2col_kernel, dim3(ew_grid((size_t)Mo * K / 4)), dim3(256), 0, s, sw.Wc, sw.Ac, wc, C, patch, stride, ho, wo);
  hipLaunchKernelGGL(im2col_kernel, dim3(ew_grid((size_t)Pn * K / 4)), dim3(256), 0, s, sw.Ws, sw.Bs, ws, C, patch, stride, rows, cols);
  hipLaunchKernelGGL(patch_axis_inv_norm_kernel, dim3(cdiv(K / 4, 64)), dim3(64), 0, s, sw.Bs, sw.inv, Pn, K);
  HIP_TRY(hipGetLastError());
  {
    GemmArgs g = {};
    g.A = sw.Ac; g.lda = K; g.a_kmajor = 0; g.a_scale_k = sw.inv; g.B = sw.Bs; g.ldb = K; g.b_kmajor = 0;
    g.M = Mo; g.N = Pn; g.K = K; g.ksplit = K; g.out32 = sw.E; g.ldo = Pn;
    if ((rc = launch_gemm(g, 1, 1, s))) return rc;
  }
  hipLaunchKernelGGL(row_argmax_kernel, dim3(Mo), dim3(64), 0, s, sw.E, sw.idx, Pn);
  HIP_TRY(hipGetLastError());
  hipLaunchKernelGGL(swap_reconstruct_kernel, dim3(ew_grid((size_t)Nc * C / 4)), dim3(256), 0, s, sw.Bs, sw.idx, sw.ss,
                     hc, wc, C, patch, stride, ho, wo);
  HIP_TRY(hipGetLastError());
  {
    GemmArgs g = {};
    g.A = sw.ss; g.lda = C; g.a_kmajor = 0; g.B = w.Tcs; g.ldb = C; g.b_kmajor = 0;
    g.M = Nc; g.N = C; g.K = C; g.ksplit = C; g.out32 = sw.col; g.ldo = C;
    if ((rc = launch_gemm(g, 1, 1, s))) return rc;
  }
  hipLaunchKernelGGL(swap_blend_kernel, dim3(ew_grid((size_t)Nc * C / 4)), dim3(256), 0, s, sw.col, content, w.mean + C,
                     (size_t)Nc * C / 4, C, alpha, out16, out32);
  HIP_TRY(hipGetLastError());
  return WCT_OK;
}
```

wct_tf_amd/csrc/wct.hip:

```cpp
#include "wct_stages.h"
#include "jacobi_dev.h"
#include "strength_rule.h"
#include <algorithm>
#include <type_traits>



template <int BC, int BP, typename Args = ApplyArgs>
__global__ __launch_bounds__(256, 2) void apply_f16x2_kernel(Args p) {
  constexpr bool SEGB = std::is_same<Args, ApplySegBatchArgs>::value;
  constexpr bool SEG = std::is_same<Args, ApplySegArgs>::value || SEGB;
  constexpr bool MAP = std::is_same<Args, ApplyMapArgs>::value;
  constexpr int TM = BC / 64, TN = BP / 64;
  constexpr int MI = BC * 4 / 256, XI = BP * 4 / 256;
  __shared__ __attribute__((aligned(16))) unsigned char lm[2][BC * 64];
  __shared__ __attribute__((aligned(16))) unsigned char lx[2][BP * 64];
  typedef unsigned int u32x4 __attribute__((ext_vector_type(4)));
  const int tid = threadIdx.x, lane = tid & 63, wave = tid >> 6;
  const int wm = wave >> 1, wn = wave & 1;
  const int pair = blockIdx.z;
  const int n0 = blockIdx.x * BP, c0 = blockIdx.y * BC;
  int seg0 = 0, N = p.N;
  [[maybe_unused]] int row0 = 0;
  if constexpr (SEGB) {
// ... 95 lines not shown
        bl[j] = *reinterpret_cast<const half8*>(lx[1] + off);
      }
#pragma unroll
      for (int i = 0; i < TM; ++i)
#pragma unroll
        for (int j = 0; j < TN; ++j) {
          acc[i][j] = __builtin_amdgcn_mfma_f32_32x32x16_f16(al[i], bh[j], acc[i][j], 0, 0, 0);
          acc[i][j] = __builtin_amdgcn_mfma_f32_32x32x16_f16(ah[i], bl[j], acc[i][j], 0, 0, 0);
          acc[i][j] = __builtin_amdgcn_mfma_f32_32x32x16_f16(ah[i], bh[j], acc[i][j], 0, 0, 0);
        }
    }
    __syncthreads();
  }

  const float inv = 1.f / (sx * sM);
  const float* bias = p.bias + (size_t)pair * C;
  const int kgrp = lane >> 5;
  f32x4 bvs[TM][4];
#pragma unroll
  for (int i = 0; i < TM; ++i)
#pragma unroll
    for (int rq = 0; rq < 4; ++rq) {
      const int co = c0 + (wm * TM + i) * 32 + 8 * rq + 4 * kgrp;
      const f32x4 z = {0.f, 0.f, 0.f, 0.f};
      bvs[i][rq] = co < C ? *reinterpret_cast<const f32x4*>(bias + co) : z;
    }
  int dst[TN];
  if constexpr (SEG)
#pragma unroll
    for (int j = 0; j < TN; ++j) {
      const int n = n0 + (wn * TN + j) * 32 + (lane & 31);
      dst[j] = p.perm[seg0 + (n < N ? n : 0)];
      if constexpr (SEGB) dst[j] += row0;
    }
  [[maybe_unused]] float amap[TN];
  [[maybe_unused]] f32x4 xv[TN][TM][4];
  if constexpr (MAP)
#pragma unroll
    for (int j = 0; j < TN; ++j) {
      const int n = n0 + (wn * TN + j) * 32 + (lane & 31), nc = n < N ? n : 0;
      const uint8_t* sm = p.smap + (size_t)pair * p.Hm * p.Wm;
      amap[j] = wct_strength_a(p.alpha, sm[wct_strength_index(nc / p.w, nc % p.w, p.stride, p.Hm, p.Wm)]);
#pragma unroll
      for (int i = 0; i < TM; ++i)
#pragma unroll
        for (int rq = 0; rq < 4; ++rq) {
          const int co = c0 + (wm * TM + i) * 32 + 8 * rq + 4 * kgrp;
          const f32x4 z = {0.f, 0.f, 0.f, 0.f};
          xv[j][i][rq] = co < C ? *reinterpret_cast<const f32x4*>(x + (size_t)nc * C + co) : z;
        }
    }
#pragma unroll
  for (int j = 0; j < TN; ++j) {
    const int n = n0 + (wn * TN + j) * 32 + (lane & 31);
    const bool n_ok = n < N;
    const size_t row = SEG ? (size_t)dst[j] * C : ((size_t)pair * N + (n_ok ? n : 0)) * C;
#pragma unroll
    for (int i = 0; i < TM; ++i) {
      const int cb = c0 + (wm * TM + i) * 32;
      unsigned pk[4][2];
#pragma unroll
      for (int rq = 0; rq < 4; ++rq) {
        const int co = cb + 8 * rq + 4 * kgrp;
        const f32x4 bv = bvs[i][rq];
        f32x4 v;
#pragma unroll
        for (int q = 0; q < 4; ++q) v[q] = acc[i][j][rq * 4 + q] * inv + bv[q];
        if constexpr (MAP)
#pragma unroll
          for (int q = 0; q < 4; ++q) v[q] = wct_strength_blend(amap[j], v[q], xv[j][i][rq][q]);
        if (p.out32 && n_ok && co < C) *reinterpret_cast<f32x4*>(p.out32 + row + co) = v;
        typedef _Float16 h2 __attribute__((ext_vector_type(2)));
        h2 lo = {(half_t)v[0], (half_t)v[1]}, hi = {(half_t)v[2], (half_t)v[3]};
        pk[rq][0] = __builtin_bit_cast(unsigned, lo);
        pk[rq][1] = __builtin_bit_cast(unsigned, hi);
      }
      if (p.out16) {
#pragma unroll
        for (int m = 0; m < 2; ++m) {
          auto sxw = __builtin_amdgcn_permlane32_swap(pk[2 * m][0], pk[2 * m + 1][0], false, false);
          auto syw = __builtin_amdgcn_permlane32_swap(pk[2 * m][1], pk[2 * m + 1][1], false, false);
          u32x4 o = {sxw[0], syw[0], sxw[1], syw[1]};
          const int co = cb + 16 * m + 8 * kgrp;
          if (n_ok && co < C) *reinterpret_cast<u32x4*>(p.out16 + row + co) = o;
        }
      }
    }
  }
}

template <typename Args>
int launch_apply_args(const Args& a, int nmax, int P, hipStream_t s) {
  const int C = a.C;
  if (C >= 128) hipLaunchKernelGGL((apply_f16x2_kernel<128, 128, Args>), dim3(cdiv(nmax, 128), cdiv(C, 128), P), dim3(256), 0, s, a);
  else hipLaunchKernelGGL((apply_f16x2_kernel<64, 128, Args>), dim3(cdiv(nmax, 128), cdiv(C, 64), P), dim3(256), 0, s, a);
  HIP_TRY(hipGetLastError());
  return WCT_OK;
}
template int launch_apply_args<ApplySegArgs>(const ApplySegArgs&, int, int, hipStream_t);
template int launch_apply_args<ApplySegBatchArgs>(const ApplySegBatchArgs&, int, int, hipStream_t);
template int launch_apply_args<ApplyMapArgs>(const ApplyMapArgs&, int, int, hipStream_t);

static int wct_nslab(int N) { int s = cdiv(N, 64); return s < 1 ? 1 : (s > 256 ? 256 : s); }

static void cov_split(int C, int Nmax, int P, int* nsplit, int* ksplit) {
  const int nt = C >= 128 ? cdiv(C, 128) : 1;
  const int tiles = nt * (nt + 1) / 2 * P;
  int want = 32 / tiles;
  if (want < 1) want = 1;
  int ks = cdiv(cdiv(Nmax, want), 32) * 32;
  if (ks < 256) ks = 256;
  *ksplit = ks;
  *nsplit = cdiv(Nmax, ks);
}

PairLayout pair_layout(int C, int Nc, int Ns) {
  PairLayout L;
  const int Nmax = Nc > Ns ? Nc : Ns;
  L.nslab = wct_nslab(Nmax);
  cov_split(C, Nmax, 1, &L.nsplit, &L.ksplit);
  return L;
}

WctCarve carve(void* base, int C, int P, const PairLayout& lay) {
  WctCarve w;
  w.nslab = lay.nslab; w.nsplit = lay.nsplit; w.ksplit = lay.ksplit;
  size_t off = 0;
  char* b = reinterpret_cast<char*>(base);
  auto take = [&](size_t bytes) { void* p = b ? b + off : nullptr; off += align_up(bytes); return p; };
  const size_t cc = (size_t)C * C * sizeof(float);
  w.mean = (float*)take((size_t)2 * P * C * sizeof(float));
  w.var = (float*)take((size_t)2 * P * C * sizeof(float));
  w.stat_partial = (float*)take((size_t)2 * P * w.nslab * C * sizeof(float));
  w.absmax = (float*)take((size_t)2 * P * w.nslab * sizeof(float));
  w.scale = (float*)take((size_t)2 * P * sizeof(float));
  w.cov_partial = (float*)take((size_t)2 * P * w.nsplit * cc);
  w.A = (float*)take(2 * P * cc);
  w.A0 = (float*)take(2 * P * cc);
  w.refresh = (int*)take((size_t)2 * P * sizeof(int));
  w.V = (float*)take(2 * P * cc);
  w.d = (float*)take((size_t)2 * P * C * sizeof(float));
  w.G = (float*)take(2 * P * cc);
  w.X = (float*)take(2 * P * cc);
  w.S2 = (float*)take(7 * P * cc);
  w.Tw = (float*)take(2 * P * cc);
  w.Tcs = w.Tw + (size_t)C * C;
  w.T = (float*)take(P * cc);
  w.M = (float*)take(P * cc);
  w.bias = (float*)take((size_t)P * C * sizeof(float));
  w.mabs = (unsigned*)take((size_t)P * sizeof(unsigned));
  w.jacobi_bytes = jacobi_workspace_bytes(C, 2 * P) + 4 * (1024 + 64 * sizeof(JacobiState));
  w.jacobi_ws = take(w.jacobi_bytes);
  w.mix = (float*)take((size_t)2 * C * sizeof(float));
  w.total = off;
  return w;
}

size_t wct_workspace_bytes(int C, int Nc, int Ns, int P) {
  const int Cw = C < 32 ? 32 : C;
  return carve(nullptr, Cw, P, pair_layout(Cw, Nc, Ns)).total;
}

int launch_blend(const WctCarve& w, int C, int P, float alpha, WctSkip skip, hipStream_t s) {
  const size_t cc = (size_t)C * C;
  GemmArgs g = {};
  g.A = w.Tcs; g.lda = C; g.a_kmajor = 0; g.B = w.Tw; g.ldb = C; g.b_kmajor = 1; g.sA = one_style(skip) ? 0 : 2 * cc; g.sB = 2 * cc;
  g.M = C; g.N = C; g.K = C; g.ksplit = C; g.out32 = w.M; g.ldo = C; g.s_out = cc;
  g.blend = 1; g.alpha = alpha; g.mabs = w.mabs;
  return launch_gemm(g, 1, P, s);
}

int launch_apply(const WctCarve& w, const float* content, int Nc, int C, int P, half_t* out16, float* out32, hipStream_t s) {
  return launch_apply_args(apply_args<ApplyArgs>(w, content, Nc, C, out16, out32), Nc, P, s);
}

static bool strength_ok(const WctStrength& sm, int Nc) {
  return sm.smap && sm.Hm >= 1 && sm.Wm >= 1 && sm.w >= 1 && sm.stride >= 1 && Nc % sm.w == 0;
}

static int launch_blend_apply_map(const WctCarve& w, const float* content, int Nc, int C, int P, WctSkip skip, const WctCall& r,
                                  const WctStrength& sm) {
  int rc;
  if ((rc = launch_blend(w, C, P, 1.f, skip, r.stream))) return rc;
  ApplyMapArgs a = apply_args<ApplyMapArgs>(w, content, Nc, C, r.out16, r.out32);
  a.smap = sm.smap; a.Hm = sm.Hm; a.Wm = sm.Wm; a.w = sm.w; a.stride = sm.stride; a.alpha = r.alpha;
  return launch_apply_args(a, Nc, P, r.stream);
}

static int launch_blend_apply(const WctCarve& w, const float* content, int Nc, int C, int P, WctSkip skip, const WctCall& r) {
  int rc;
  if ((rc = launch_blend(w, C, P, r.alpha, skip, r.stream))) return rc;
  return launch_apply(w, content, Nc, C, P, r.out16, r.out32, r.stream);
}

WctStyleKey wct_style_key(int C, int Nc, int Ns) {
  const PairLayout L = pair_layout(std::max(C, 32), Nc, Ns);
  return WctStyleKey{L.nslab, L.nsplit, L.ksplit};
}
size_t wct_style_state_floats(int C) { return (size_t)2 * C + (size_t)C * C; }

template <typename Ref>
__global__ __launch_bounds__(256) void style_load_kernel(Ref r, float* mean, float* var, float* Tw, int C, int with_T) {
  const int k = blockIdx.y;
  const float* src = r.state[k];
  const size_t cc = (size_t)C * C, n = (size_t)2 * C + (with_T ? cc : 0), slot = (size_t)(2 * k + 1);
  for (size_t i = (blockIdx.x * (size_t)blockDim.x + threadIdx.x) * 4; i < n; i += (size_t)gridDim.x * blockDim.x * 4) {
    const f32x4 v = *reinterpret_cast<const f32x4*>(src + i);
    float* dst = i < (size_t)C ? mean + slot * C + i : (i < (size_t)2 * C ? var + slot * C + (i - C) : Tw + slot * cc + (i - 2 * C));
    *reinterpret_cast<f32x4*>(dst) = v;
  }
}

template <typename Ref>
static int launch_style_load(const Ref& r, int K, const WctCarve& w, int C, bool with_T, hipStream_t s) {
  for (int k = 0; k < K; ++k) ARG_CHECK(r.state[k] != nullptr);
  const size_t n4 = ((size_t)2 * C + (with_T ? (size_t)C * C : 0)) / 4;
  hipLaunchKernelGGL(style_load_kernel<Ref>, dim3((unsigned)std::min<size_t>((n4 + 255) / 256, 256), K), dim3(256), 0, s, r, w.mean, w.var,
                     w.Tw, C, with_T ? 1 : 0);
  HIP_TRY(hipGetLastError());
  return WCT_OK;
}

int launch_style_load_slots(const WctStyleSlots& r, int P, const WctCarve& w, int C, bool with_T, hipStream_t s) {
  ARG_CHECK(P >= 1 && P <= WCT_PLAN_PAIRS);
  return launch_style_load(r, P, w, C, with_T, s);
}

static void style_plan(SlotPlan* sp, void* base, int C, const float* style, int Ns, const WctStyleKey& key) {
  *sp = SlotPlan{};
  sp->P = 1; sp->skip = WCT_SKIP_CONTENT; sp->nwhite = 0;
  sp->slot[1] = {style, Ns, PairLayout{key.nslab, key.nsplit, key.ksplit}};
  plan_carve(sp, base, C);
}

size_t wct_style_workspace_bytes(int C, int Ns, const WctStyleKey& key) {
  SlotPlan sp;
  style_plan(&sp, nullptr, C, nullptr, Ns, key);
  return sp.total;
}

int launch_style_state(const float* style, int Ns, int C, const WctStyleKey& key, int adain, const WctCall& r, float* state) {
  const int mode = r.mode; hipStream_t s = r.stream;
  ARG_CHECK(style && state && C % 32 == 0 && C >= 32 && C <= 1024 && Ns >= (adain ? 1 : 2) && launch_map_fits((size_t)Ns * C, 4));
  ARG_CHECK(adain || mode == WCT_MODE_NP || mode == WCT_MODE_TF);
  ARG_CHECK(key.nslab >= 1 && key.nslab <= 256 && key.nsplit >= 1 && key.ksplit >= 256 && key.ksplit % 32 == 0 &&
            (long long)key.nsplit * key.ksplit >= Ns);
  SlotPlan sp;
  style_plan(&sp, r.workspace, C, style, Ns, key);
  ARG_CHECK(r.workspace_bytes >= sp.total);
  const WctCarve& w = sp.w;
  int rc;
  if (adain) {
    if ((rc = launch_plan_stats(sp, C, true, false, 0.f, s))) return rc;
    HIP_TRY(hipMemcpyAsync(state + C, w.var + C, (size_t)C * sizeof(float), hipMemcpyDeviceToDevice, s));
  } else {
    if ((rc = launch_plan_stats(sp, C, false, true, cov_eps(mode, r.eps), s))) return rc;
    if ((rc = launch_eig_stage(w, C, sp.P, sp.skip, 1, nullptr, r.eig_fail, s))) return rc;
    if ((rc = launch_spectral_tail(w, C, sp.P, 1.f, mode, r.eps, sp.skip, sp.nwhite, s))) return rc;
    HIP_TRY(hipMemcpyAsync(state + 2 * C, w.Tw + (size_t)C * C, (size_t)C * C * sizeof(float), hipMemcpyDeviceToDevice, s));
  }
  HIP_TRY(hipMemcpyAsync(state, w.mean + C, (size_t)C * sizeof(float), hipMemcpyDeviceToDevice, s));
  return WCT_OK;
}

int launch_wct(const float* content, int Nc, const float* style, int Ns, int C, int P, WctSkip skip, const WctCall& r,
               const WctFeatStats* stats, const WctStyleRef* prep, const WctWarmRef* warm, const WctStrength* sm) {
  const int mode = r.mode, stages = r.stages; hipStream_t s = r.stream;
  ARG_CHECK(C % 32 == 0 && C >= 32 && C <= 1024 && Nc >= 2 && Ns >= 2 && P >= 1 && P <= 32);
  ARG_CHECK(!sm || strength_ok(*sm, Nc));
  ARG_CHECK(skip == WCT_SKIP_NONE || skip == WCT_SKIP_SHARED_STYLE);
  ARG_CHECK(!warm || (warm->basis && (skip == WCT_SKIP_NONE || prep)));
  if (prep) skip = WCT_SKIP_STYLE;
  ARG_CHECK(mode == WCT_MODE_NP || mode == WCT_MODE_TF);
  ARG_CHECK(launch_map_fits((size_t)Nc * C, 4) && launch_map_fits((size_t)Ns * C, 4));
  WctCarve w = carve(r.workspace, C, P, pair_layout(C, Nc, Ns));
  ARG_CHECK(r.workspace_bytes >= w.total);
  int rc;
  if (stages & WCT_STAGE_COV) {
    if ((rc = launch_means(content, Nc, style, Ns, C, P, w, false, skip, s, stats))) return rc;
    if ((rc = launch_cov(content, Nc, style, Ns, C, P, w, cov_eps(mode, r.eps), skip, s))) return rc;
  }
  if (stages & WCT_STAGE_EIG) {
    const bool rotate = warm && warm->valid;
    if (rotate && (rc = launch_warm_rotate(w, C, P, warm->basis, s))) return rc;
    if ((rc = launch_eig_stage(w, C, P, skip, (stages & WCT_STAGE_EIG_FP32UPDATE) ? 0 : 1, r.sweeps_dev, r.eig_fail, s, rotate ? 0 : 2)))
      return rc;
    if (rotate && (rc = launch_warm_compose(w, C, P, warm->basis, s))) return rc;
    if (warm && (rc = launch_warm_store(w.V + (size_t)2 * (P - 1) * C * C, w.X, warm->basis, C, s))) return rc;
  }
  if (!(stages & WCT_STAGE_APPLY)) return WCT_OK;

  if (prep && (rc = launch_style_load(*prep, 1, w, C, true, s))) return rc;
  if ((rc = launch_spectral_tail(w, C, P, sm ? 1.f : r.alpha, mode, r.eps, skip, P, s))) return rc;
  if (sm) return launch_blend_apply_map(w, content, Nc, C, P, skip, r, *sm);
  return launch_blend_apply(w, content, Nc, C, P, skip, r);
}

void plan_carve(SlotPlan* sp, void* base, int C) {
  PairLayout mx = {1, 1, 0};
  for (int m = 0; m < 2 * sp->P; ++m)
    if (sp->slot[m].n) { mx.nslab = std::max(mx.nslab, sp->slot[m].lay.nslab); mx.nsplit = std::max(mx.nsplit, sp->slot[m].lay.nsplit); }
  sp->w = carve(base, C, std::max(sp->P, 1), mx);
  sp->total = sp->w.total;
}

bool plan_fits(const SlotPlan& sp, int C) {
  for (int m = 0; m < 2 * sp.P; ++m)
    if (!launch_map_fits((size_t)sp.slot[m].n * C, 4)) return false;
  return true;
}

static bool mix_plan(SlotPlan* sp, void* base, int C, const float* content, int Nc, const float* const* styles, const int* Ns,
                     int K, const float* lambda, int nmin, const WctFeatStats* stats, bool prepared = false) {
  if (!Ns || !lambda || K < 1 || K > WCT_MIX_MAX) return false;
  int ref = 0;
  for (int k = 0; k < K; ++k) {
    if ((styles && !styles[k]) || Ns[k] < nmin || !(lambda[k] >= 0.f && lambda[k] <= 1.f)) return false;
// ... 189 lines not shown
```

wct_tf_amd/csrc/wct_stages.h:

```cpp
#pragma once
#include "common.h"


constexpr int EIG_CORRECT = 2;
constexpr float JACOBI_TOL_FN = 1.5e-2f;
constexpr float JACOBI_TOL_FN2 = 4e-2f;
constexpr float JACOBI_TOL_FN_WCT = EIG_CORRECT >= 2 ? JACOBI_TOL_FN2 : (EIG_CORRECT ? JACOBI_TOL_FN : 0.f);

static inline size_t align_up(size_t x) { return (x + 255) & ~(size_t)255; }

struct WctCarve {
  float *mean, *var, *stat_partial, *absmax, *scale, *cov_partial, *A, *A0, *V, *d, *G, *X, *S2, *Tw, *Tcs, *T, *M, *bias, *mix;
  unsigned* mabs; int* refresh;
  void* jacobi_ws; size_t jacobi_bytes;
  int nslab, nsplit, ksplit;
  size_t total;
};

struct PairLayout { int nslab, nsplit, ksplit; };
PairLayout pair_layout(int C, int Nc, int Ns);
WctCarve carve(void* base, int C, int P, const PairLayout& lay);

static inline float cov_eps(int mode, float eps_in) {
  return mode == WCT_MODE_TF ? (eps_in >= 0.f ? eps_in : 1e-8f) : 0.f;
}

static inline unsigned rows_grid(size_t N, int C) {
  const size_t blocks = (N * C / 4 + 255) / 256;
  return (unsigned)(blocks > 2048 ? 2048 : blocks);
}

constexpr int WCT_PLAN_PAIRS = 32;
struct SlotPlan {
  int P; WctSkip skip; int nwhite;
  struct Slot { const float* x; int n; PairLayout lay; } slot[2 * WCT_PLAN_PAIRS];
  const float* u0; const unsigned* umax0;
  WctCarve w;
  size_t total;
};
void plan_carve(SlotPlan* sp, void* base, int C);
bool plan_fits(const SlotPlan& sp, int C);

struct ApplyArgs {
  const float* x; int N; int C;
  const float* mean;
  const float* M; const float* bias;
  const float* xscale;
  const unsigned* mabs;
  half_t* out16; float* out32;
};
struct ApplySegArgs : ApplyArgs { const int* seg_off; const int* perm; int lab[WCT_MIX_MAX]; };
struct ApplySegBatchArgs : ApplyArgs { const int* seg_off; const int* perm; unsigned char fl[WCT_PLAN_PAIRS]; };
struct ApplyMapArgs : ApplyArgs { const uint8_t* smap; int Hm, Wm, w, stride; float alpha; };
template <typename Args>
static inline Args apply_args(const WctCarve& w, const float* x, int N, int C, half_t* out16, float* out32) {
  Args a;
  a.x = x; a.N = N; a.C = C; a.mean = w.mean; a.M = w.M; a.bias = w.bias;
  a.xscale = w.scale; a.mabs = w.mabs; a.out16 = out16; a.out32 = out32;
  return a;
}
__device__ __host__ __forceinline__ int seg_frame(unsigned char fl) { return fl >> 3; }
__device__ __host__ __forceinline__ int seg_label(unsigned char fl) { return fl & 7; }

int launch_means(const float* content, int Nc, const float* style, int Ns, int C, int P, const WctCarve& w, bool with_var,
                 WctSkip skip, hipStream_t s, const WctFeatStats* fs);
int launch_cov(const float* content, int Nc, const float* style, int Ns, int C, int P, const WctCarve& w, float eps, WctSkip skip,
               hipStream_t s);
int launch_plan_stats(const SlotPlan& sp, int C, bool with_var, bool with_cov, float eps, hipStream_t s);
int launch_eig_stage(const WctCarve& w, int C, int P, WctSkip skip, int u_f16, int* sweeps_dev, int* eig_fail, hipStream_t s,
                     int check_from = 2);
int launch_spectral_tail(const WctCarve& w, int C, int P, float alpha, int mode, float eps_in, WctSkip skip, int nwhite, hipStream_t s);
int launch_spectral_tail_refreshed(const WctCarve& w, int C, int P, float alpha, int mode, float eps_in, WctSkip skip, int nwhite,
                                   hipStream_t s);
int launch_blend(const WctCarve& w, int C, int P, float alpha, WctSkip skip, hipStream_t s);
int launch_apply(const WctCarve& w, const float* content, int Nc, int C, int P, half_t* out16, float* out32, hipStream_t s);
template <typename Args> int launch_apply_args(const Args& a, int nmax, int P, hipStream_t s);
int launch_warm_rotate(const WctCarve& w, int C, int P, const float* V0, hipStream_t s);
int launch_warm_compose(const WctCarve& w, int C, int P, const float* V0, hipStream_t s);
int launch_warm_store(const float* V, float* scratch, float* basis, int C, hipStream_t s);
int launch_style_load_slots(const WctStyleSlots& r, int P, const WctCarve& w, int C, bool with_T, hipStream_t s);
```

Before: 687.4.

## Run spectral and blend matrix products as split-f16 MFMA GEMMs

For channel counts of at least 256 (divisible by 128), the CxC matrix products in the spectral tail and the blend step now go through a split-precision scheme. Each fp32 matrix is scaled by a per-matrix power of two derived from per-tile absmax words, split into high and low f16 planes, and multiplied with three f16 MFMA products per tile pair (hi*hi, hi*lo, lo*hi). This replaces the fp32 GEMM path for those products to use matrix cores while keeping close to fp32 accuracy. It adds absmax and split kernels, extra workspace for the planes, and absmax tracking inside the spectral kernels. Style-swap keeps fp32 products, and a test entry point is exposed.

```diff
diff --git a/include/wct_hip.h b/include/wct_hip.h
--- a/include/wct_hip.h
+++ b/include/wct_hip.h
@@ -64,6 +64,8 @@
                 const float* bias, int Cout, int relu, int upsample, float* y);
 int wct_conv3x3_f16(wct_ctx* ctx, const float* x, int B, int H, int W, int Cin, const float* w_hwio,
                     const float* bias, int Cout, int relu, int upsample, int pool, int algo, float* y);
+int wct_spectral_product(wct_ctx* ctx, const float* A, const float* A_odd, const float* B, int nbatch, int n, int a_kmajor,
+                         int b_kmajor, int skip, int blend, float alpha, int algo, float* out, float* mabs_out);
 int wct_maxpool(wct_ctx* ctx, const float* x, int H, int W, int C, float* y);
 int wct_encode(wct_ctx* ctx, const float* img01, int H, int W, int level, float* feat);
 int wct_decode(wct_ctx* ctx, const float* feat, int h, int w, int level, float* img);
diff --git a/wct_tf_amd/_lib.py b/wct_tf_amd/_lib.py
--- a/wct_tf_amd/_lib.py
+++ b/wct_tf_amd/_lib.py
@@ -36,6 +36,7 @@
     ('wct_eigh', C.c_int, [_P, _F, C.c_int, C.c_int, _F, _F, _I]),
     ('wct_conv3x3', C.c_int, [_P, _F, C.c_int, C.c_int, C.c_int, _F, _F, C.c_int, C.c_int, C.c_int, _F]),
     ('wct_conv3x3_f16', C.c_int, [_P, _F, C.c_int, C.c_int, C.c_int, C.c_int, _F, _F, C.c_int, C.c_int, C.c_int, C.c_int, C.c_int, _F]),
+    ('wct_spectral_product', C.c_int, [_P, _F, _F, _F, C.c_int, C.c_int, C.c_int, C.c_int, C.c_int, C.c_int, C.c_float, C.c_int, _F, _F]),
     ('wct_maxpool', C.c_int, [_P, _F, C.c_int, C.c_int, C.c_int, _F]),
     ('wct_encode', C.c_int, [_P, _F, C.c_int, C.c_int, C.c_int, _F]),
     ('wct_decode', C.c_int, [_P, _F, C.c_int, C.c_int, C.c_int, _F]),
diff --git a/wct_tf_amd/context.py b/wct_tf_amd/context.py
--- a/wct_tf_amd/context.py
+++ b/wct_tf_amd/context.py
@@ -505,6 +505,17 @@
         check(self.lib.wct_conv3x3_f16(self.h, fptr(x), n, h, wd, cin, fptr(w), fptr(b), cout, int(relu), int(upsample), int(pool),
                                        int(algo), fptr(y)))
         return y[0] if single else y
+
+    def spectral_product(self, a, b, algo, a_odd=None, a_kmajor=False, b_kmajor=True, skip=0, blend=None):
+        a, b = f32(a), f32(b)
+        nb, n, _ = b.shape
+        ao = None if a_odd is None else f32(a_odd)
+        out = np.empty((nb, n, n), np.float32)
+        mabs = np.zeros(nb, np.float32)
+        check(self.lib.wct_spectral_product(self.h, fptr(a), None if ao is None else fptr(ao), fptr(b), nb, n, int(a_kmajor),
+                                            int(b_kmajor), int(skip), int(blend is not None), float(blend or 0.0), int(algo),
+                                            fptr(out), fptr(mabs)))
+        return (out, mabs) if blend is not None else out
 
     def maxpool(self, x):
         x = f32(x)
diff --git a/wct_tf_amd/csrc/api_ops.hip b/wct_tf_amd/csrc/api_ops.hip
--- a/wct_tf_amd/csrc/api_ops.hip
+++ b/wct_tf_amd/csrc/api_ops.hip
@@ -400,6 +400,65 @@
   return rc;
 }
 
+extern "C" int wct_spectral_product(wct_ctx* c, const float* A, const float* A_odd, const float* B, int nbatch, int n, int a_kmajor,
+                                    int b_kmajor, int skip, int blend, float alpha, int algo, float* out, float* mabs_out) {
+  ARG_CHECK(c && A && B && out && nbatch >= 1 && nbatch <= 64 && n >= 64 && n <= 1024 && n % 64 == 0 && (algo == 1 || algo == 2));
+  ARG_CHECK(skip >= WCT_SKIP_NONE && skip <= WCT_SKIP_STYLES && (!blend || mabs_out) && (algo == 1 || n % 128 == 0));
+  HIP_TRY(hipSetDevice(c->device));
+  const size_t nn = (size_t)n * n, pp = 2 * nn;
+  const int nA = A_odd ? (nbatch + 1) / 2 : nbatch, nAo = A_odd ? nbatch / 2 : 0;
+  void *dA, *dB, *dAo = nullptr;
+  TRY(stage_in(c, 0, A, nA * nn * 4, &dA));
+  TRY(stage_in(c, 1, B, nbatch * nn * 4, &dB));
+  if (nAo) TRY(stage_in(c, 2, A_odd, nAo * nn * 4, &dAo));
+  const size_t out_b = nbatch * nn * 4, pl_b = pp * sizeof(half_t);
+  const size_t S = (size_t)(n / 64) * (n / 64);
+  TRY(ensure(c, c->wct_ws, out_b + (nA + nAo + nbatch) * pl_b + (3 * 64 * S + 64) * sizeof(float)));
+  char* ws = (char*)c->wct_ws.p;
+  float* dout = (float*)ws;
+  half_t* pA = (half_t*)(ws + out_b);
+  half_t* pAo = (half_t*)((char*)pA + nA * pl_b);
+  half_t* pB = (half_t*)((char*)pAo + nAo * pl_b);
+  float* words = (float*)((char*)pB + nbatch * pl_b);
+  float *wA = words, *wAo = words + 64 * S, *wB = words + 128 * S;
+  unsigned* mabs = (unsigned*)(words + 192 * S);
+  hipStream_t s = c->stream;
+  HIP_TRY(hipMemsetAsync(dout, 0, nbatch * nn * 4, s));
+  HIP_TRY(hipMemsetAsync(mabs, 0, 64 * sizeof(unsigned), s));
+  const bool odd_given = dAo != nullptr;
+  if (algo == 1) {
+    GemmArgs g = {};
+    g.A = (float*)dA; g.lda = n; g.a_kmajor = a_kmajor; g.B = (float*)dB; g.ldb = n; g.b_kmajor = b_kmajor;
+    g.M = g.N = g.K = g.ksplit = g.ldo = n; g.sA = g.sB = g.s_out = nn; g.out32 = dout; g.skip = (WctSkip)skip;
+    if (odd_given) { g.A_odd = (float*)dAo; g.sA_odd = nn; }
+    g.blend = blend; g.alpha = alpha; g.mabs = mabs;
+    TRY(launch_gemm(g, 1, nbatch, s));
+  } else {
+    TRY(launch_plane_absmax((float*)dA, nn, n, wA, S, nA, WCT_SKIP_NONE, s));
+    if (odd_given) TRY(launch_plane_absmax((float*)dAo, nn, n, wAo, S, nAo, WCT_SKIP_NONE, s));
+    TRY(launch_plane_absmax((float*)dB, nn, n, wB, S, nbatch, WCT_SKIP_NONE, s));
+    auto split = [&](const void* src, const float* word, half_t* planes, bool turn, int nb) {
+      PlaneSplitArgs a = {};
+      a.src = (const float*)src; a.s_src = nn; a.rows = a.cols = n; a.word = word; a.s_word = S; a.nslot = (int)S;
+      (turn ? a.transposed : a.straight) = planes;
+      a.skip = WCT_SKIP_NONE;
+      return launch_plane_split(a, nb, s);
+    };
+    TRY(split(dA, wA, pA, a_kmajor != 0, nA));
+    if (odd_given) TRY(split(dAo, wAo, pAo, a_kmajor != 0, nAo));
+    TRY(split(dB, wB, pB, b_kmajor != 0, nbatch));
+    PlaneGemmArgs g = {};
+    g.A = pA; g.sA = pp; g.wA = wA; g.swA = S; g.nslot = (int)S;
+    if (odd_given) { g.A_odd = pAo; g.sA_odd = pp; g.wA_odd = wAo; g.swA_odd = S; }
+    g.B = pB; g.sB = pp; g.wB = wB; g.swB = S;
+    g.M = g.N = g.K = g.ldo = n; g.out = dout; g.s_out = nn; g.skip = (WctSkip)skip;
+    g.blend = blend; g.alpha = alpha; g.mabs = mabs;
+    TRY(launch_plane_gemm(g, nbatch, s));
+  }
+  if (mabs_out) HIP_TRY(hipMemcpyAsync(mabs_out, mabs, nbatch * sizeof(float), hipMemcpyDeviceToHost, s));
+  return fetch(c, out, dout, nbatch * nn * 4);
+}
+
 extern "C" int wct_maxpool(wct_ctx* c, const float* x, int H, int W, int C, float* y) {
   ARG_CHECK(c && x && y && C % 8 == 0);
   HIP_TRY(hipSetDevice(c->device));
diff --git a/wct_tf_amd/csrc/common.h b/wct_tf_amd/csrc/common.h
--- a/wct_tf_amd/csrc/common.h
+++ b/wct_tf_amd/csrc/common.h
@@ -143,6 +143,29 @@
 };
 
 int launch_gemm(GemmArgs g, int nsplit, int nbatch, hipStream_t s);
+
+static inline bool planes_take(int C) { return C >= 256 && C % 128 == 0; }
+struct PlaneSplitArgs {
+  const float* src; size_t s_src; int rows, cols;
+  const float* word; size_t s_word; int nslot;
+  half_t* straight; int straight_odd;
+  half_t* transposed; int transposed_even;
+  WctSkip skip;
+};
+struct PlaneGemmArgs {
+  const half_t* A; size_t sA; const float* wA; size_t swA;
+  const half_t* A_odd; size_t sA_odd; const float* wA_odd; size_t swA_odd;
+  const half_t* B; size_t sB; const float* wB; size_t swB;
+  int nslot;
+  int M, N, K;
+  float* out; size_t s_out; int ldo;
+  float* omax;
+  WctSkip skip;
+  int blend; float alpha; unsigned* mabs;
+};
+int launch_plane_absmax(const float* src, size_t s_src, int C, float* word, size_t s_word, int nb, WctSkip skip, hipStream_t s);
+int launch_plane_split(const PlaneSplitArgs& a, int nb, hipStream_t s);
+int launch_plane_gemm(const PlaneGemmArgs& g, int nbatch, hipStream_t s);
 
 enum { WCT_MODE_NP = 0, WCT_MODE_TF = 1 };
 
diff --git a/wct_tf_amd/csrc/spectral.hip b/wct_tf_amd/csrc/spectral.hip
--- a/wct_tf_amd/csrc/spectral.hip
+++ b/wct_tf_amd/csrc/spectral.hip
@@ -52,6 +52,7 @@
   const float *X1, *X2;
   int C; float shift; int correct, second; WctSkip skip;
   unsigned* mabs; const float* mean; float* bias; float alpha; int mode;
+  float *mxN, *mxG, *mxR, *mxP;
 };
 
 __global__ __launch_bounds__(256) void spectral_open_all_kernel(SpecAllArgs a) {
@@ -76,6 +77,7 @@
   spectral_tile_load(t, Am, C, p0, q0, tid);
   __syncthreads();
   const int ty = tid >> 4, tx = tid & 15;
+  float mg = 0.f, mn = 0.f, mr = 0.f, mp = 0.f;
 #pragma unroll
   for (int i = 0; i < 4; ++i) {
     const int pl = ty * 4 + i, p = p0 + pl, q = q0 + tx * 4;
@@ -100,6 +102,24 @@
     if (a.second) {
       *reinterpret_cast<f32x4*>(a.N + m * cc + o) = n4;
       if (kind == 0) { *reinterpret_cast<f32x4*>(a.R + pair * cc + o) = r4; *reinterpret_cast<f32x4*>(a.Pm + pair * cc + o) = p4; }
+    }
+    if (a.mxG)
+#pragma unroll
+      for (int j = 0; j < 4; ++j) {
+        mg = fmaxf(mg, fabsf(g[j])); mn = fmaxf(mn, fabsf(n4[j])); mr = fmaxf(mr, fabsf(r4[j])); mp = fmaxf(mp, fabsf(p4[j]));
+      }
+  }
+  if (a.mxG) {
+    __shared__ float mred[4][4];
+    mg = wave_max(mg); mn = wave_max(mn); mr = wave_max(mr); mp = wave_max(mp);
+    if ((tid & 63) == 0) { mred[0][tid >> 6] = mg; mred[1][tid >> 6] = mn; mred[2][tid >> 6] = mr; mred[3][tid >> 6] = mp; }
+    __syncthreads();
+    if (tid < 4) {
+      const float v = fmaxf(fmaxf(mred[tid][0], mred[tid][1]), fmaxf(mred[tid][2], mred[tid][3]));
+      const size_t S = (size_t)gridDim.x * gridDim.y, slot = (size_t)blockIdx.y * gridDim.x + blockIdx.x;
+      if (tid == 0) a.mxG[m * S + slot] = v;
+      else if (a.second && tid == 1) a.mxN[m * S + slot] = v;
+      else if (a.second && kind == 0) (tid == 2 ? a.mxR : a.mxP)[pair * S + slot] = v;
     }
   }
 }
@@ -138,6 +158,7 @@
     for (int j = 0; j < 4; ++j) { x2t[ty * 4 + i][tx * 4 + j] = v2[j]; x1t[ty * 4 + i][tx * 4 + j] = v1[j]; }
   }
   __syncthreads();
+  float mg = 0.f;
 #pragma unroll
   for (int i = 0; i < 4; ++i) {
     const int pl = ty * 4 + i, p = p0 + pl, q = q0 + tx * 4;
@@ -159,6 +180,15 @@
       g[j] += l2;
     }
     *reinterpret_cast<f32x4*>(Gm + o) = g;
+#pragma unroll
+    for (int j = 0; j < 4; ++j) mg = fmaxf(mg, fabsf(g[j]));
+  }
+  if (a.mxG) {
+    __shared__ float mred[4];
+    mg = wave_max(mg);
+    if ((tid & 63) == 0) mred[tid >> 6] = mg;
+    __syncthreads();
+    if (tid == 0) a.mxG[((size_t)m * gridDim.y + blockIdx.y) * gridDim.x + blockIdx.x] = fmaxf(fmaxf(mred[0], mred[1]), fmaxf(mred[2], mred[3]));
   }
 }
 
@@ -179,21 +209,56 @@
   return launch_gemm(r2, 1, 2 * P, s);
 }
 
+static int split_level(const float* src, size_t s_src, int C, const float* word, half_t* straight, int straight_odd,
+                       half_t* transposed, WctSkip skip, int nb, hipStream_t s) {
+  PlaneSplitArgs a = {};
+  a.src = src; a.s_src = s_src; a.rows = a.cols = C; a.word = word; a.s_word = plane_slots(C); a.nslot = plane_slots(C);
+  a.straight = straight; a.straight_odd = straight_odd; a.transposed = transposed; a.skip = skip;
+  return launch_plane_split(a, nb, s);
+}
+static PlaneGemmArgs level_plane_product(int C, WctSkip skip) {
+  PlaneGemmArgs g = {};
+  g.M = g.N = g.K = g.ldo = C; g.s_out = (size_t)C * C; g.skip = skip; g.nslot = plane_slots(C);
+  return g;
+}
+
 int launch_spectral_tail_refreshed(const WctCarve& w, int C, int P, float alpha, int mode, float eps_in, WctSkip skip, int nwhite,
-                                   hipStream_t s) {
+                                   hipStream_t s, bool fp32_products) {
   int rc;
   const size_t cc = (size_t)C * C;
   const float shift = mode == WCT_MODE_NP ? (eps_in >= 0.f ? eps_in : 1e-5f) : 0.f;
   const int second = EIG_CORRECT >= 2;
+  const bool planes = planes_take(C) && !fp32_products && w.planes;
+  const size_t pp = 2 * cc;
+  const PlaneWords mx = plane_words(w.pmax, P, C);
+  const size_t S = plane_slots(C);
+  half_t* const pl = w.planes;
   const dim3 tiles(cdiv(C, 64), cdiv(C, 64), 2 * P);
   SpecAllArgs sa = {};
   sa.A = w.A; sa.G = w.G; sa.C = C; sa.shift = shift; sa.correct = EIG_CORRECT; sa.second = second; sa.skip = skip;
   sa.N = w.S2; float* X2 = sa.N + 2 * P * cc; sa.R = X2 + 2 * P * cc; sa.Pm = sa.R + P * cc; float* X1 = sa.Pm + P * cc;
   sa.X1 = X1; sa.X2 = X2;
   sa.mabs = w.mabs; sa.mean = w.mean; sa.bias = w.bias; sa.alpha = alpha; sa.mode = mode;
+  if (planes) { sa.mxN = mx.N; sa.mxG = mx.G; sa.mxR = mx.R; sa.mxP = mx.Pm; }
   hipLaunchKernelGGL(spectral_open_all_kernel, tiles, dim3(256), 0, s, sa);
   HIP_TRY(hipGetLastError());
-  if (second) {
+  if (second && planes) {
+    half_t *NT = pl, *Ns = pl + 2 * P * pp, *Rp = pl + 3 * P * pp, *Pp = pl + 4 * P * pp;
+    if ((rc = split_level(sa.N, cc, C, mx.N, Ns, 1, NT, skip, 2 * P, s))) return rc;
+    if (nwhite > 0 && (rc = split_level(sa.Pm, cc, C, mx.Pm, Pp, 0, nullptr, WCT_SKIP_NONE, nwhite, s))) return rc;
+    PlaneGemmArgs a = level_plane_product(C, skip);
+    a.A = Pp; a.sA = pp; a.wA = mx.Pm; a.swA = S; a.A_odd = Ns; a.sA_odd = pp; a.wA_odd = mx.N + S; a.swA_odd = 2 * S;
+    a.B = NT; a.sB = pp; a.wB = mx.N; a.swB = S; a.out = X2;
+    if ((rc = launch_plane_gemm(a, 2 * P, s))) return rc;
+    if (nwhite > 0) {
+      if ((rc = split_level(sa.R, cc, C, mx.R, Rp, 0, nullptr, WCT_SKIP_NONE, nwhite, s))) return rc;
+      PlaneGemmArgs b = level_plane_product(C, WCT_SKIP_NONE);
+      b.A = Rp; b.sA = pp; b.wA = mx.R; b.swA = S; b.B = NT; b.sB = 2 * pp; b.wB = mx.N; b.swB = 2 * S; b.out = X1;
+      if ((rc = launch_plane_gemm(b, nwhite, s))) return rc;
+    }
+    hipLaunchKernelGGL(spectral_add2_all_kernel, tiles, dim3(256), 0, s, sa);
+    HIP_TRY(hipGetLastError());
+  } else if (second) {
     GemmArgs a = level_product(C, skip);
     a.A = sa.Pm; a.A_odd = sa.N + cc; a.sA_odd = 2 * cc; a.a_kmajor = 0; a.B = sa.N; a.b_kmajor = 1; a.out32 = X2;
     if ((rc = launch_gemm(a, 1, 2 * P, s))) return rc;
@@ -203,6 +268,18 @@
     hipLaunchKernelGGL(spectral_add2_all_kernel, tiles, dim3(256), 0, s, sa);
     HIP_TRY(hipGetLastError());
   }
+  if (planes) {
+    half_t *GT = pl, *Vp = pl + 2 * P * pp, *Xp = pl + 4 * P * pp;
+    if ((rc = split_level(w.G, cc, C, mx.G, nullptr, 0, GT, skip, 2 * P, s))) return rc;
+    if ((rc = split_level(w.V, cc, C, nullptr, Vp, 0, nullptr, skip, 2 * P, s))) return rc;
+    PlaneGemmArgs g = level_plane_product(C, skip);
+    g.A = Vp; g.sA = pp; g.B = GT; g.sB = pp; g.wB = mx.G; g.swB = S; g.out = w.X; g.omax = mx.X;
+    if ((rc = launch_plane_gemm(g, 2 * P, s))) return rc;
+    if ((rc = split_level(w.X, cc, C, mx.X, Xp, 0, nullptr, skip, 2 * P, s))) return rc;
+    PlaneGemmArgs h = level_plane_product(C, skip);
+    h.A = Xp; h.sA = pp; h.wA = mx.X; h.swA = S; h.B = Vp; h.sB = pp; h.out = w.Tw;
+    return launch_plane_gemm(h, 2 * P, s);
+  }
   GemmArgs g = level_product(C, skip);
   g.A = w.V; g.a_kmajor = 0; g.B = w.G; g.b_kmajor = 1; g.out32 = w.X;
   if ((rc = launch_gemm(g, 1, 2 * P, s))) return rc;
@@ -212,7 +289,7 @@
 }
 
 int launch_spectral_tail(const WctCarve& w, int C, int P, float alpha, int mode, float eps_in, WctSkip skip, int nwhite,
-                         hipStream_t s) {
+                         hipStream_t s, bool fp32_products) {
   const int rc = launch_refresh(w, C, P, skip, s);
-  return rc ? rc : launch_spectral_tail_refreshed(w, C, P, alpha, mode, eps_in, skip, nwhite, s);
-}
+  return rc ? rc : launch_spectral_tail_refreshed(w, C, P, alpha, mode, eps_in, skip, nwhite, s, fp32_products);
+}
diff --git a/wct_tf_amd/csrc/stats_gemm.hip b/wct_tf_amd/csrc/stats_gemm.hip
--- a/wct_tf_amd/csrc/stats_gemm.hip
+++ b/wct_tf_amd/csrc/stats_gemm.hip
@@ -564,3 +564,212 @@
   }
   return WCT_OK;
 }
+
+__device__ __forceinline__ int plane_exp(const float* slots, int nslot, int lane) {
+  if (!slots) return 14;
+  float m = 0.f;
+  for (int i = lane; i < nslot; i += 64) m = fmaxf(m, slots[i]);
+  m = wave_max(m);
+  if (!(m > 0.f) || !(m < __builtin_inff())) return 0;
+  int e;
+  frexpf(m, &e);
+  e = 14 - e;
+  return e > 100 ? 100 : (e < -100 ? -100 : e);
+}
+
+__global__ __launch_bounds__(256) void plane_absmax_kernel(const float* src, size_t s_src, float* word, size_t s_word, int skip) {
+  __shared__ float red[4];
+  const int b = blockIdx.y, tid = threadIdx.x;
+  if (skip_style_mat(b, skip)) return;
+  const f32x4* x = reinterpret_cast<const f32x4*>(src + b * s_src) + (size_t)blockIdx.x * 1024;
+  float av = 0.f;
+#pragma unroll
+  for (int i = 0; i < 4; ++i) {
+    const f32x4 v = x[tid + i * 256];
+    av = fmaxf(fmaxf(av, fmaxf(fabsf(v[0]), fabsf(v[1]))), fmaxf(fabsf(v[2]), fabsf(v[3])));
+  }
+  av = wave_max(av);
+  if ((tid & 63) == 0) red[tid >> 6] = av;
+  __syncthreads();
+  if (tid == 0) word[b * s_word + blockIdx.x] = fmaxf(fmaxf(red[0], red[1]), fmaxf(red[2], red[3]));
+}
+
+__global__ __launch_bounds__(256) void plane_split_kernel(PlaneSplitArgs a) {
+  __shared__ __attribute__((aligned(8))) half_t tt[2][64][68];
+  const int b = blockIdx.z, r0 = blockIdx.y * 64, c0 = blockIdx.x * 64, tid = threadIdx.x, ty = tid >> 4, tx = tid & 15;
+  if (skip_style_mat(b, a.skip)) return;
+  const size_t rc = (size_t)a.rows * a.cols;
+  const float* src = a.src + b * a.s_src;
+  const float sc = ldexpf(1.f, plane_exp(a.word ? a.word + b * a.s_word : nullptr, a.nslot, tid & 63));
+  half_t* st = a.straight && (!a.straight_odd || (b & 1)) ? a.straight + (size_t)(a.straight_odd ? b >> 1 : b) * 2 * rc : nullptr;
+  half_t* tr = a.transposed && (!a.transposed_even || !(b & 1)) ? a.transposed + (size_t)(a.transposed_even ? b >> 1 : b) * 2 * rc : nullptr;
+#pragma unroll
+  for (int i = 0; i < 4; ++i) {
+    const int r = ty * 4 + i;
+    const size_t o = (size_t)(r0 + r) * a.cols + c0 + tx * 4;
+    const f32x4 v = *reinterpret_cast<const f32x4*>(src + o);
+    half4 h, l;
+#pragma unroll
+    for (int j = 0; j < 4; ++j) {
+      const float s = v[j] * sc;
+      h[j] = (half_t)s;
+      l[j] = (half_t)(s - (float)h[j]);
+    }
+    if (st) { *reinterpret_cast<half4*>(st + o) = h; *reinterpret_cast<half4*>(st + rc + o) = l; }
+    if (tr)
+#pragma unroll
+      for (int j = 0; j < 4; ++j) { tt[0][tx * 4 + j][r] = h[j]; tt[1][tx * 4 + j][r] = l[j]; }
+  }
+  if (!tr) return;
+  __syncthreads();
+#pragma unroll
+  for (int i = 0; i < 4; ++i) {
+    const int c = ty * 4 + i;
+    const size_t o = (size_t)(c0 + c) * a.rows + r0 + tx * 4;
+    *reinterpret_cast<half4*>(tr + o) = *reinterpret_cast<const half4*>(&tt[0][c][tx * 4]);
+    *reinterpret_cast<half4*>(tr + rc + o) = *reinterpret_cast<const half4*>(&tt[1][c][tx * 4]);
+  }
+}
+
+__global__ __launch_bounds__(256, 2) void gemm_planes_kernel(PlaneGemmArgs p) {
+  typedef unsigned int u32x4 __attribute__((ext_vector_type(4)));
+  __shared__ __attribute__((aligned(16))) unsigned char la[2][128 * 64];
+  __shared__ __attribute__((aligned(16))) unsigned char lb[2][128 * 64];
+  const int tid = threadIdx.x, lane = tid & 63, wave = tid >> 6;
+  const int wm = wave >> 1, wn = wave & 1;
+  const int m0 = blockIdx.y * 128, n0 = blockIdx.x * 128, batch = blockIdx.z;
+  if (skip_style_mat(batch, p.skip)) return;
+  const half_t* A; const float* wa;
+  if (p.A_odd) {
+    A = (batch & 1) ? p.A_odd + (batch >> 1) * p.sA_odd : p.A + (batch >> 1) * p.sA;
+    wa = (batch & 1) ? p.wA_odd + (batch >> 1) * p.swA_odd : (p.wA ? p.wA + (batch >> 1) * p.swA : nullptr);
+  } else {
+    A = p.A + batch * p.sA;
+    wa = p.wA ? p.wA + batch * p.swA : nullptr;
+  }
+  const half_t* B = p.B + batch * p.sB;
+  const int ea = plane_exp(wa, p.nslot, lane), eb = plane_exp(p.wB ? p.wB + batch * p.swB : nullptr, p.nslot, lane);
+  const int K = p.K;
+  const size_t pa = (size_t)p.M * K, pb = (size_t)p.N * K;
+
+  const half_t* ap[2]; const half_t* bp[2];
+  int off[2];
+#pragma unroll
+  for (int i = 0; i < 2; ++i) {
+    const int item = tid + i * 256, row = item >> 2, kq = item & 3;
+    ap[i] = A + (size_t)(m0 + row) * K + kq * 8;
+    bp[i] = B + (size_t)(n0 + row) * K + kq * 8;
+    off[i] = (row * 4 + (kq ^ ((row >> 2) & 3))) * 16;
+  }
+
+  f32x16 acc[2][2];
+#pragma unroll
+  for (int i = 0; i < 2; ++i)
+#pragma unroll
+    for (int j = 0; j < 2; ++j)
+#pragma unroll
+      for (int r = 0; r < 16; ++r) acc[i][j][r] = 0.f;
+
+  u32x4 ra[2][2], rb[2][2];
+  auto load = [&](int k0) {
+#pragma unroll
+    for (int i = 0; i < 2; ++i) {
+      ra[i][0] = *reinterpret_cast<const u32x4*>(ap[i] + k0);
+      ra[i][1] = *reinterpret_cast<const u32x4*>(ap[i] + pa + k0);
+      rb[i][0] = *reinterpret_cast<const u32x4*>(bp[i] + k0);
+      rb[i][1] = *reinterpret_cast<const u32x4*>(bp[i] + pb + k0);
+    }
+  };
+  load(0);
+  for (int k0 = 0; k0 < K; k0 += 32) {
+#pragma unroll
+    for (int i = 0; i < 2; ++i) {
+      *reinterpret_cast<u32x4*>(la[0] + off[i]) = ra[i][0];
+      *reinterpret_cast<u32x4*>(la[1] + off[i]) = ra[i][1];
+      *reinterpret_cast<u32x4*>(lb[0] + off[i]) = rb[i][0];
+      *reinterpret_cast<u32x4*>(lb[1] + off[i]) = rb[i][1];
+    }
+    __syncthreads();
+    if (k0 + 32 < K) load(k0 + 32);
+#pragma unroll
+    for (int ks = 0; ks < 2; ++ks) {
+      const int chunk = ks * 2 + (lane >> 5);
+      half8 ah[2], al[2], bh[2], bl[2];
+#pragma unroll
+      for (int i = 0; i < 2; ++i) {
+        const int r = (wm * 2 + i) * 32 + (lane & 31);
+        const int o = (r * 4 + (chunk ^ ((r >> 2) & 3))) * 16;
+        ah[i] = *reinterpret_cast<const half8*>(la[0] + o);
+        al[i] = *reinterpret_cast<const half8*>(la[1] + o);
+      }
+#pragma unroll
+      for (int j = 0; j < 2; ++j) {
+        const int r = (wn * 2 + j) * 32 + (lane & 31);
+        const int o = (r * 4 + (chunk ^ ((r >> 2) & 3))) * 16;
+        bh[j] = *reinterpret_cast<const half8*>(lb[0] + o);
+        bl[j] = *reinterpret_cast<const half8*>(lb[1] + o);
+      }
+#pragma unroll
+      for (int i = 0; i < 2; ++i)
+#pragma unroll
+        for (int j = 0; j < 2; ++j) {
+          acc[i][j] = __builtin_amdgcn_mfma_f32_32x32x16_f16(al[i], bh[j], acc[i][j], 0, 0, 0);
+          acc[i][j] = __builtin_amdgcn_mfma_f32_32x32x16_f16(ah[i], bl[j], acc[i][j], 0, 0, 0);
+          acc[i][j] = __builtin_amdgcn_mfma_f32_32x32x16_f16(ah[i], bh[j], acc[i][j], 0, 0, 0);
+        }
+    }
+    __syncthreads();
+  }
+
+  const float ia = ldexpf(1.f, -ea), ib = ldexpf(1.f, -eb);
+  float* out = p.out + batch * p.s_out;
+  float av = 0.f;
+#pragma unroll
+  for (int i = 0; i < 2; ++i)
+#pragma unroll
+    for (int j = 0; j < 2; ++j) {
+      const int gn = n0 + (wn * 2 + j) * 32 + (lane & 31);
+#pragma unroll
+      for (int r = 0; r < 16; ++r) {
+        const int gm = m0 + (wm * 2 + i) * 32 + (r & 3) + 8 * (r >> 2) + 4 * (lane >> 5);
+        float v = acc[i][j][r] * ia * ib;
+        if (p.blend) {
+          v = p.alpha * v;
+          if (gm == gn) v += 1.f - p.alpha;
+        }
+        av = fmaxf(av, fabsf(v));
+        out[(size_t)gm * p.ldo + gn] = v;
+      }
+    }
+  if (p.blend) {
+    for (int o = 32; o > 0; o >>= 1) av = fmaxf(av, __shfl_xor(av, o, 64));
+    if (lane == 0 && av < 1e30f) atomicMax(p.mabs + batch, __float_as_uint(av));
+  } else if (p.omax) {
+    av = wave_max(av);
+    const int nsx = p.N >> 6;
+    if (lane == 0) p.omax[(size_t)batch * (p.M >> 6) * nsx + (size_t)(blockIdx.y * 2 + wm) * nsx + blockIdx.x * 2 + wn] = av;
+  }
+}
+
+int launch_plane_absmax(const float* src, size_t s_src, int C, float* word, size_t s_word, int nb, WctSkip skip, hipStream_t s) {
+  ARG_CHECK(src && word && C >= 64 && C % 64 == 0 && nb >= 1);
+  hipLaunchKernelGGL(plane_absmax_kernel, dim3((C / 64) * (C / 64), nb), dim3(256), 0, s, src, s_src, word, s_word, (int)skip);
+  HIP_TRY(hipGetLastError());
+  return WCT_OK;
+}
+
+int launch_plane_split(const PlaneSplitArgs& a, int nb, hipStream_t s) {
+  ARG_CHECK(a.src && (a.straight || a.transposed) && a.rows >= 64 && a.cols >= 64 && a.rows % 64 == 0 && a.cols % 64 == 0 && nb >= 1);
+  hipLaunchKernelGGL(plane_split_kernel, dim3(a.cols / 64, a.rows / 64, nb), dim3(256), 0, s, a);
+  HIP_TRY(hipGetLastError());
+  return WCT_OK;
+}
+
+int launch_plane_gemm(const PlaneGemmArgs& g, int nbatch, hipStream_t s) {
+  ARG_CHECK(g.A && g.B && g.out && g.M >= 128 && g.N >= 128 && g.K >= 32 && g.M % 128 == 0 && g.N % 128 == 0 && g.K % 32 == 0 &&
+            g.ldo >= g.N && nbatch >= 1 && (!g.blend || g.mabs) && (!g.A_odd || g.wA_odd) &&
+            ((!g.wA && !g.wB && !g.wA_odd) || g.nslot >= 1));
+  hipLaunchKernelGGL(gemm_planes_kernel, dim3(g.N / 128, g.M / 128, nbatch), dim3(256), 0, s, g);
+  HIP_TRY(hipGetLastError());
+  return WCT_OK;
+}
diff --git a/wct_tf_amd/csrc/style_swap.hip b/wct_tf_amd/csrc/style_swap.hip
--- a/wct_tf_amd/csrc/style_swap.hip
+++ b/wct_tf_amd/csrc/style_swap.hip
@@ -149,10 +149,10 @@
   r.stages = WCT_STAGE_COV | WCT_STAGE_EIG | WCT_STAGE_EIG_FP32UPDATE; r.eig_fail = eig_fail; r.stream = s;
   if ((rc = launch_wct(content, Nc, style, Ns, C, 1, WCT_SKIP_NONE, r, nullptr, nullptr, nullptr))) return rc;
   const size_t cc = (size_t)C * C;
-  if ((rc = launch_spectral_tail(w, C, 1, alpha, WCT_MODE_TF, eps, WCT_SKIP_NONE, 1, s))) return rc;
+  if ((rc = launch_spectral_tail(w, C, 1, alpha, WCT_MODE_TF, eps, WCT_SKIP_NONE, 1, s, true))) return rc;
   WctCarve v = w;
   v.A += cc; v.V += cc; v.G += cc; v.X += cc; v.Tw = w.T;
-  if ((rc = launch_spectral_tail_refreshed(v, C, 1, alpha, WCT_MODE_TF, eps, WCT_SKIP_STYLE, 1, s))) return rc;
+  if ((rc = launch_spectral_tail_refreshed(v, C, 1, alpha, WCT_MODE_TF, eps, WCT_SKIP_STYLE, 1, s, true))) return rc;
   auto apply = [&](const float* X, int N, const float* mean, const float* T, float* out) {
     GemmArgs g = {};
     g.A = X; g.lda = C; g.a_kmajor = 0; g.a_sub_k = mean; g.B = T; g.ldb = C; g.b_kmajor = 0;
diff --git a/wct_tf_amd/csrc/wct.hip b/wct_tf_amd/csrc/wct.hip
--- a/wct_tf_amd/csrc/wct.hip
+++ b/wct_tf_amd/csrc/wct.hip
@@ -271,6 +271,8 @@
   w.jacobi_bytes = jacobi_workspace_bytes(C, 2 * P) + 4 * (1024 + 64 * sizeof(JacobiState));
   w.jacobi_ws = take(w.jacobi_bytes);
   w.mix = (float*)take((size_t)2 * C * sizeof(float));
+  w.planes = planes_take(C) ? (half_t*)take((size_t)6 * P * 2 * C * C * sizeof(half_t)) : nullptr;
+  w.pmax = planes_take(C) ? (float*)take((size_t)10 * P * plane_slots(C) * sizeof(float)) : nullptr;
   w.total = off;
   return w;
 }
@@ -282,6 +284,24 @@
 
 int launch_blend(const WctCarve& w, int C, int P, float alpha, WctSkip skip, hipStream_t s) {
   const size_t cc = (size_t)C * C;
+  if (planes_take(C) && w.planes) {
+    int rc;
+    const size_t pp = 2 * cc;
+    const PlaneWords mx = plane_words(w.pmax, P, C);
+    const size_t S = plane_slots(C);
+    const WctSkip live = one_style(skip) ? WCT_SKIP_SHARED_STYLE : WCT_SKIP_NONE;
+    if ((rc = launch_plane_absmax(w.Tw, cc, C, mx.T, S, 2 * P, live, s))) return rc;
+    PlaneSplitArgs sp = {};
+    sp.src = w.Tw; sp.s_src = cc; sp.rows = sp.cols = C; sp.word = mx.T; sp.s_word = S; sp.nslot = (int)S;
+    sp.transposed = w.planes; sp.transposed_even = 1; sp.straight = w.planes + P * pp; sp.straight_odd = 1; sp.skip = live;
+    if ((rc = launch_plane_split(sp, 2 * P, s))) return rc;
+    PlaneGemmArgs g = {};
+    g.A = w.planes + P * pp; g.sA = one_style(skip) ? 0 : pp; g.wA = mx.T + S; g.swA = one_style(skip) ? 0 : 2 * S;
+    g.B = w.planes; g.sB = pp; g.wB = mx.T; g.swB = 2 * S; g.nslot = (int)S;
+    g.M = g.N = g.K = g.ldo = C; g.out = w.M; g.s_out = cc; g.skip = WCT_SKIP_NONE;
+    g.blend = 1; g.alpha = alpha; g.mabs = w.mabs;
+    return launch_plane_gemm(g, P, s);
+  }
   GemmArgs g = {};
   g.A = w.Tcs; g.lda = C; g.a_kmajor = 0; g.B = w.Tw; g.ldb = C; g.b_kmajor = 1; g.sA = one_style(skip) ? 0 : 2 * cc; g.sB = 2 * cc;
   g.M = C; g.N = C; g.K = C; g.ksplit = C; g.out32 = w.M; g.ldo = C; g.s_out = cc;
diff --git a/wct_tf_amd/csrc/wct_stages.h b/wct_tf_amd/csrc/wct_stages.h
--- a/wct_tf_amd/csrc/wct_stages.h
+++ b/wct_tf_amd/csrc/wct_stages.h
@@ -9,9 +9,21 @@
 
 static inline size_t align_up(size_t x) { return (x + 255) & ~(size_t)255; }
 
+static inline int plane_slots(int C) { return (C / 64) * (C / 64); }
+struct PlaneWords { float *N, *G, *X, *R, *Pm, *T; };
+static inline PlaneWords plane_words(float* pmax, int P, int C) {
+  const size_t S = plane_slots(C);
+  return PlaneWords{pmax, pmax + 2 * P * S, pmax + 4 * P * S, pmax + 6 * P * S, pmax + 7 * P * S, pmax + 8 * P * S};
+}
+__device__ __forceinline__ float wave_max(float av) {
+  for (int o = 32; o > 0; o >>= 1) av = fmaxf(av, __shfl_xor(av, o, 64));
+  return av;
+}
+
 struct WctCarve {
   float *mean, *var, *stat_partial, *absmax, *scale, *cov_partial, *A, *A0, *V, *d, *G, *X, *S2, *Tw, *Tcs, *T, *M, *bias, *mix;
   unsigned* mabs; int* refresh;
+  half_t* planes; float* pmax;
   void* jacobi_ws; size_t jacobi_bytes;
   int nslab, nsplit, ksplit;
   size_t total;
@@ -69,9 +81,10 @@
 int launch_plan_stats(const SlotPlan& sp, int C, bool with_var, bool with_cov, float eps, hipStream_t s);
 int launch_eig_stage(const WctCarve& w, int C, int P, WctSkip skip, int u_f16, int* sweeps_dev, int* eig_fail, hipStream_t s,
                      int check_from = 2);
-int launch_spectral_tail(const WctCarve& w, int C, int P, float alpha, int mode, float eps_in, WctSkip skip, int nwhite, hipStream_t s);
+int launch_spectral_tail(const WctCarve& w, int C, int P, float alpha, int mode, float eps_in, WctSkip skip, int nwhite, hipStream_t s,
+                         bool fp32_products = false);
 int launch_spectral_tail_refreshed(const WctCarve& w, int C, int P, float alpha, int mode, float eps_in, WctSkip skip, int nwhite,
-                                   hipStream_t s);
+                                   hipStream_t s, bool fp32_products = false);
 int launch_blend(const WctCarve& w, int C, int P, float alpha, WctSkip skip, hipStream_t s);
 int launch_apply(const WctCarve& w, const float* content, int Nc, int C, int P, half_t* out16, float* out32, hipStream_t s);
 template <typename Args> int launch_apply_args(const Args& a, int nmax, int P, hipStream_t s);
```

Measured after the change: 693.7, median of 6. About the same (+0.9%).
